# bastienjacquet/CudaDepthMapIntegration

Measured on AMD Instinct MI355X. Metric: Gvoxel-projections/s, higher is better.
Workload: dtype f64

## Files before the change

cudadepthmapintegration_amd/capi.py:

```python
from __future__ import annotations

import ctypes
import os
import sys
from typing import NamedTuple

import numpy as np

from . import build as _build
from .scene import GridDesc, RayPotential, Views

DMI_OK = 0
DMI_F32, DMI_F64 = 0, 1
DMI_DEPTH_AUTO, DMI_DEPTH_F32, DMI_DEPTH_F64 = 0, 1, 2
DMI_COMPONENTS_MIN_TRIANGLES, DMI_COMPONENTS_LARGEST = 0, 1

VARIANT_EXACT_DIVISION = 1
VARIANT_GENERAL_K = 2
VARIANT_FORCE_GENERAL = 16
VARIANT_NO_BRICK_CLASSES = 256
VARIANT_KEEP_BEHIND_ADDS = 1024
VARIANT_NO_INTERIOR = 2048
VARIANT_XCD_RUNS = 8192
VARIANT_ZMAJOR_SLOTS = 16384
VARIANT_PERSISTENT_ALWAYS = 32768
VARIANT_PERSISTENT_NEVER = 65536
VARIANT_NO_WINDOWS = 262144
VARIANT_WINDOWS_ALWAYS = 524288
VARIANT_COST_ORDER = 1048576
VARIANT_NO_COST_ORDER = 2097152
VARIANT_BRICK_CLASSES_ALWAYS = 131072
VARIANT_FIXED_TILE_SHAPE = 4096
VARIANT_SPATIAL_ORDER = 512
VARIANT_TILE_SHAPE = {"tk16_w5_g8_1x1": 0, "tk8_w6_g8_2x2": 32, "tk16_w5_g8_2x2": 64, "tk8_w6": 96, "tk8_w7_g8": 128, "tk16_w5_g4": 160,
                      "tk16_w6_g2": 192, "tk8_w6_g8_1x1": 224}


class GridDescC(ctypes.Structure):
    _fields_ = [("cell_dims", ctypes.c_int32 * 3), ("origin", ctypes.c_double * 3),
                ("spacing", ctypes.c_double * 3), ("grid_matrix", ctypes.c_double * 16)]


class RayPotentialC(ctypes.Structure):
    _fields_ = [("thickness", ctypes.c_double), ("rho", ctypes.c_double), ("eta", ctypes.c_double),
                ("delta", ctypes.c_double)]


class OptionsC(ctypes.Structure):
    _fields_ = [("device", ctypes.c_int32), ("grid_dtype", ctypes.c_int32), ("depth_storage", ctypes.c_int32),
                ("count_hits", ctypes.c_int32), ("kernel_variant", ctypes.c_int32), ("z_first", ctypes.c_int32),
                ("stream", ctypes.c_void_p), ("external_grid", ctypes.c_void_p)]


class TimingsC(ctypes.Structure):
    _fields_ = [("last_fuse_kernel_ms", ctypes.c_double), ("total_fuse_kernel_ms", ctypes.c_double),
                ("fuse_launches", ctypes.c_uint64), ("last_upload_ms", ctypes.c_double),
                ("last_download_ms", ctypes.c_double), ("last_cell_to_point_ms", ctypes.c_double),
                ("last_fuse_main_kernel_ms", ctypes.c_double), ("total_fuse_main_kernel_ms", ctypes.c_double)]


class InfoC(ctypes.Structure):
    _fields_ = [("n_voxels", ctypes.c_int64), ("n_views", ctypes.c_int32), ("depth_width", ctypes.c_int32),
                ("depth_height", ctypes.c_int32), ("depth_storage_in_use", ctypes.c_int32),
                ("grid_dtype", ctypes.c_int32), ("k_mode", ctypes.c_int32), ("kernel_variant", ctypes.c_int32),
                ("tiled_kernel", ctypes.c_int32), ("device_bytes", ctypes.c_uint64), ("pixels_without_depth", ctypes.c_uint64)]


class MultiOptionsC(ctypes.Structure):
    _fields_ = [("grid_dtype", ctypes.c_int32), ("depth_storage", ctypes.c_int32), ("kernel_variant", ctypes.c_int32),
                ("partition", ctypes.c_int32), ("exchange", ctypes.c_int32), ("n_slabs", ctypes.c_int32)]


class MultiInfoC(ctypes.Structure):
    _fields_ = [("world", ctypes.c_int32), ("n_local", ctypes.c_int32), ("first_rank", ctypes.c_int32),
                ("rccl_ranks", ctypes.c_int32), ("rccl_version", ctypes.c_int32), ("partition", ctypes.c_int32),
                ("exchange", ctypes.c_int32), ("n_slabs", ctypes.c_int32), ("n_voxels", ctypes.c_int64),
                ("n_views_total", ctypes.c_int64), ("n_views_local", ctypes.c_int64)]


class MultiTimingsC(ctypes.Structure):
    _fields_ = [("last_step_ms", ctypes.c_double), ("last_fuse_kernel_ms", ctypes.c_double),
                ("total_step_ms", ctypes.c_double), ("steps", ctypes.c_uint64)]


DMI_PARTITION_VIEWS, DMI_PARTITION_Z_SLABS = 0, 1
DMI_EXCHANGE_ALL_REDUCE, DMI_EXCHANGE_REDUCE_SCATTER, DMI_EXCHANGE_PEER_COPY = 0, 1, 2
DMI_UNIQUE_ID_BYTES = 128

ABI_SYMBOLS = [
    "dmi_default_options", "dmi_create", "dmi_destroy", "dmi_last_error", "dmi_add_views", "dmi_add_views_f32",
    "dmi_clear_views", "dmi_reset_grid", "dmi_upload_grid", "dmi_fuse", "dmi_fuse_range", "dmi_fuse_slab", "dmi_fuse_range_download", "dmi_synchronize",
    "dmi_download_grid_f64", "dmi_download_grid_f32", "dmi_download_hits", "dmi_grid_device_pointer",
    "dmi_get_brick_class_histogram", "dmi_get_timings", "dmi_get_info", "dmi_alloc_pinned", "dmi_free_pinned", "dmi_pcie_probe", "dmi_fp64_probe", "dmi_abi_version", "dmi_device_count",
    "dmi_color_mesh", "dmi_color_last_error", "dmi_cell_to_point", "dmi_download_point_data_f64",
    "dmi_point_data_device_pointer", "dmi_color_create", "dmi_color_destroy", "dmi_color_add_views",
    "dmi_color_clear_views", "dmi_color_process", "dmi_color_get_kernel_ms", "dmi_get_mixed_reason_histogram", "dmi_get_window_pair_count", "dmi_get_view_paths", "dmi_get_upload_kernel_ms", "dmi_sizeof_info", "dmi_sizeof_timings",
    "dmi_color_set_scratch_budget", "dmi_color_set_vertex_reorder", "dmi_color_add_views_with_depth", "dmi_color_set_depth_test",
    "dmi_iso_active_cells",
    "dmi_extract_isosurface", "dmi_download_isosurface", "dmi_get_isosurface_kernel_ms",
    "dmi_extract_isosurface_normals", "dmi_download_isosurface_normals",
    "dmi_filter_isosurface_components", "dmi_download_isosurface_regions", "dmi_get_isosurface_filter_kernel_ms",
    "dmi_get_isosurface_filter_pass_ms", "dmi_get_isosurface_filter_cas_retries",
    "dmi_smooth_isosurface", "dmi_get_isosurface_smooth_kernel_ms", "dmi_get_isosurface_smooth_pass_ms",
    "dmi_multi_default_options", "dmi_multi_view_shard", "dmi_multi_z_slab", "dmi_multi_slab_ranges", "dmi_multi_peer_chunk", "dmi_multi_create",
    "dmi_multi_get_unique_id", "dmi_multi_create_rank", "dmi_multi_destroy", "dmi_multi_last_error", "dmi_multi_add_views",
    "dmi_multi_add_views_f32", "dmi_multi_add_local_views", "dmi_multi_add_local_views_f32", "dmi_multi_clear_views", "dmi_multi_fuse", "dmi_multi_synchronize",
    "dmi_multi_download_grid_f32", "dmi_multi_download_grid_f64", "dmi_multi_get_info", "dmi_multi_get_timings",
    "dmi_multi_local_context",
]

_lib = None


class DmiError(RuntimeError):
    def __init__(self, code: int, message: str):
        super().__init__(f"dmi error {code}: {message}")
        self.code = code


def library_path() -> str:
    return _build.LIB_PATH


def load() -> ctypes.CDLL:
    global _lib
    if _lib is not None:
        return _lib
    if "torch" not in sys.modules:
        try:
            import torch
        except Exception:
            pass
    path = _build.build()
    if not os.path.exists(path):
        raise RuntimeError(f"{path} is missing: the HIP extension is required, there is no CPU fallback")
    L = ctypes.CDLL(path)
    vp, i32, dbl = ctypes.c_void_p, ctypes.c_int32, ctypes.c_double
    dp = ctypes.POINTER(ctypes.c_double)
    L.dmi_default_options.argtypes = [ctypes.POINTER(OptionsC)]
    L.dmi_default_options.restype = None
    L.dmi_create.argtypes = [ctypes.POINTER(GridDescC), ctypes.POINTER(RayPotentialC), ctypes.POINTER(OptionsC),
                             ctypes.POINTER(vp)]
    L.dmi_destroy.argtypes = [vp]
    L.dmi_destroy.restype = None
    L.dmi_last_error.argtypes = [vp]
    L.dmi_last_error.restype = ctypes.c_char_p
    L.dmi_add_views.argtypes = [vp, dp, dp, dbl, dp, dp, i32, i32, i32]
    L.dmi_add_views_f32.argtypes = [vp, ctypes.POINTER(ctypes.c_float), dp, dp, i32, i32, i32]
    L.dmi_clear_views.argtypes = [vp]
    L.dmi_reset_grid.argtypes = [vp]
    L.dmi_upload_grid.argtypes = [vp, dp]
    L.dmi_fuse.argtypes = [vp]
    L.dmi_fuse_range.argtypes = [vp, i32, i32]
    L.dmi_fuse_slab.argtypes = [vp, i32, i32]
    if hasattr(L, "dmi_fuse_range_download"):
        L.dmi_fuse_range_download.argtypes = [vp, i32, i32, vp, i32, i32]
    L.dmi_synchronize.argtypes = [vp]
    L.dmi_download_grid_f64.argtypes = [vp, dp]
    L.dmi_download_grid_f32.argtypes = [vp, ctypes.POINTER(ctypes.c_float)]
    L.dmi_download_hits.argtypes = [vp, ctypes.POINTER(ctypes.c_uint32), ctypes.POINTER(ctypes.c_uint64)]
    L.dmi_grid_device_pointer.argtypes = [vp, ctypes.POINTER(vp)]
    L.dmi_cell_to_point.argtypes = [vp]
    L.dmi_download_point_data_f64.argtypes = [vp, dp]
    L.dmi_point_data_device_pointer.argtypes = [vp, ctypes.POINTER(vp)]
    if hasattr(L, "dmi_iso_active_cells"):
        L.dmi_iso_active_cells.argtypes = [vp, ctypes.c_double, ctypes.POINTER(ctypes.c_uint64), ctypes.POINTER(ctypes.c_int64),
                                           ctypes.c_uint64]
    if hasattr(L, "dmi_extract_isosurface"):
        L.dmi_extract_isosurface.argtypes = [vp, ctypes.c_double, ctypes.POINTER(ctypes.c_uint64), ctypes.POINTER(ctypes.c_uint64)]
        L.dmi_download_isosurface.argtypes = [vp, dp, ctypes.POINTER(ctypes.c_int64)]
        L.dmi_get_isosurface_kernel_ms.argtypes = [vp, dp]
    if hasattr(L, "dmi_extract_isosurface_normals"):
        L.dmi_extract_isosurface_normals.argtypes = [vp, ctypes.c_double, ctypes.POINTER(ctypes.c_uint64), ctypes.POINTER(ctypes.c_uint64)]
        L.dmi_download_isosurface_normals.argtypes = [vp, ctypes.POINTER(ctypes.c_float)]
    if hasattr(L, "dmi_filter_isosurface_components"):
        u64p = ctypes.POINTER(ctypes.c_uint64)
        L.dmi_filter_isosurface_components.argtypes = [vp, ctypes.c_int, ctypes.c_uint64, u64p, u64p, u64p, u64p]
        L.dmi_download_isosurface_regions.argtypes = [vp, ctypes.POINTER(ctypes.c_int64), ctypes.POINTER(ctypes.c_int64)]
        L.dmi_get_isosurface_filter_kernel_ms.argtypes = [vp, dp]
        L.dmi_get_isosurface_filter_pass_ms.argtypes = [vp, dp]
        L.dmi_get_isosurface_filter_cas_retries.argtypes = [vp, u64p]
    if hasattr(L, "dmi_smooth_isosurface"):
        L.dmi_smooth_isosurface.argtypes = [vp, i32, dbl, dbl]
        L.dmi_get_isosurface_smooth_kernel_ms.argtypes = [vp, dp]
        L.dmi_get_isosurface_smooth_pass_ms.argtypes = [vp, dp]
    L.dmi_get_brick_class_histogram.argtypes = [vp, ctypes.POINTER(ctypes.c_uint64)]
    L.dmi_get_mixed_reason_histogram.argtypes = [vp, ctypes.POINTER(ctypes.c_uint64)]
    if hasattr(L, "dmi_get_window_pair_count"):
        L.dmi_get_window_pair_count.argtypes = [vp, ctypes.POINTER(ctypes.c_uint64)]
    if hasattr(L, "dmi_get_view_paths"):
        L.dmi_get_view_paths.argtypes = [vp, ctypes.POINTER(ctypes.c_uint64)]
    if hasattr(L, "dmi_get_upload_kernel_ms"):
        L.dmi_get_upload_kernel_ms.argtypes = [vp, dp, dp]
    for name in ("dmi_sizeof_info", "dmi_sizeof_timings"):
        if hasattr(L, name):
            getattr(L, name).restype = ctypes.c_size_t
    L.dmi_get_timings.argtypes = [vp, ctypes.POINTER(TimingsC)]
    L.dmi_get_info.argtypes = [vp, ctypes.POINTER(InfoC)]
    L.dmi_alloc_pinned.argtypes = [ctypes.c_size_t, ctypes.POINTER(vp)]
    L.dmi_free_pinned.argtypes = [vp]
    L.dmi_pcie_probe.argtypes = [i32, ctypes.c_size_t, dp, dp]
    L.dmi_fp64_probe.argtypes = [i32, ctypes.c_double, dp]
    u8p = ctypes.POINTER(ctypes.c_uint8)
    L.dmi_color_mesh.argtypes = [dp, ctypes.c_int64, u8p, dp, dp, i32, i32, i32, i32, u8p, u8p, ctypes.POINTER(ctypes.c_int32)]
    L.dmi_color_create.argtypes = [i32, ctypes.POINTER(vp)]
    L.dmi_color_destroy.argtypes = [vp]
    L.dmi_color_destroy.restype = None
    L.dmi_color_add_views.argtypes = [vp, u8p, dp, dp, i32, i32, i32]
    L.dmi_color_clear_views.argtypes = [vp]
    L.dmi_color_process.argtypes = [vp, dp, ctypes.c_int64, u8p, u8p, ctypes.POINTER(ctypes.c_int32)]
    L.dmi_color_get_kernel_ms.argtypes = [vp, dp]
    L.dmi_color_set_scratch_budget.argtypes = [vp, ctypes.c_uint64]
    L.dmi_color_set_vertex_reorder.argtypes = [vp, i32]
    L.dmi_color_add_views_with_depth.argtypes = [vp, u8p, dp, dp, dp, i32, i32, i32]
    L.dmi_color_set_depth_test.argtypes = [vp, i32, ctypes.c_double]
    L.dmi_color_last_error.argtypes = []
    L.dmi_color_last_error.restype = ctypes.c_char_p
    i64, i64p, i32p = ctypes.c_int64, ctypes.POINTER(ctypes.c_int64), ctypes.POINTER(ctypes.c_int32)
    L.dmi_multi_default_options.argtypes = [ctypes.POINTER(MultiOptionsC)]
    L.dmi_multi_default_options.restype = None
    L.dmi_multi_view_shard.argtypes = [i64, i32, i32, i64p, i64p]
    L.dmi_multi_z_slab.argtypes = [i32, i32, i32, i32p, i32p]
    L.dmi_multi_slab_ranges.argtypes = [i32, i32, i32p, i32p, i32]
    if hasattr(L, "dmi_multi_peer_chunk"):
        L.dmi_multi_peer_chunk.argtypes = [i64, i32, i32, i64p, i64p]
    L.dmi_multi_create.argtypes = [ctypes.POINTER(GridDescC), ctypes.POINTER(RayPotentialC), ctypes.POINTER(MultiOptionsC),
                                   i32p, i32, ctypes.POINTER(vp)]
    L.dmi_multi_get_unique_id.argtypes = [u8p]
    L.dmi_multi_create_rank.argtypes = [ctypes.POINTER(GridDescC), ctypes.POINTER(RayPotentialC), ctypes.POINTER(MultiOptionsC),
                                        i32, i32, i32, u8p, ctypes.POINTER(vp)]
    L.dmi_multi_destroy.argtypes = [vp]
    L.dmi_multi_destroy.restype = None
    L.dmi_multi_last_error.argtypes = [vp]
    L.dmi_multi_last_error.restype = ctypes.c_char_p
    L.dmi_multi_add_views.argtypes = [vp, dp, dp, dbl, dp, dp, i32, i32, i32]
    L.dmi_multi_add_views_f32.argtypes = [vp, ctypes.POINTER(ctypes.c_float), dp, dp, i32, i32, i32]
    L.dmi_multi_add_local_views.argtypes = [vp, i32, dp, dp, dbl, dp, dp, i32, i32, i32]
    L.dmi_multi_add_local_views_f32.argtypes = [vp, i32, ctypes.POINTER(ctypes.c_float), dp, dp, i32, i32, i32]
    L.dmi_multi_clear_views.argtypes = [vp]
    L.dmi_multi_fuse.argtypes = [vp]
    L.dmi_multi_synchronize.argtypes = [vp]
    L.dmi_multi_download_grid_f32.argtypes = [vp, ctypes.POINTER(ctypes.c_float), i64p, i64p]
    L.dmi_multi_download_grid_f64.argtypes = [vp, dp, i64p, i64p]
    L.dmi_multi_get_info.argtypes = [vp, ctypes.POINTER(MultiInfoC)]
    L.dmi_multi_get_timings.argtypes = [vp, ctypes.POINTER(MultiTimingsC)]
    L.dmi_multi_local_context.argtypes = [vp, i32, ctypes.POINTER(vp)]
    from . import build as _b
    for name in ABI_SYMBOLS:
        if _b.LIB_OVERRIDE and not hasattr(L, name):
            continue
        fn = getattr(L, name)
        if fn.restype is ctypes.c_int:
            fn.restype = ctypes.c_int
    _lib = L
    return L


def pinned_empty(shape, dtype) -> np.ndarray:
    L = load()
    n = int(np.prod(shape)) * np.dtype(dtype).itemsize
    p = ctypes.c_void_p()
    rc = L.dmi_alloc_pinned(n, ctypes.byref(p))
    if rc != DMI_OK:
        raise DmiError(rc, "dmi_alloc_pinned failed")
    buf = (ctypes.c_char * n).from_address(p.value)
    return np.frombuffer(buf, dtype=dtype).reshape(shape)


def pcie_probe(device: int = 0, n_bytes: int = 256 << 20) -> tuple[float, float]:
    L = load()
    a, b = ctypes.c_double(), ctypes.c_double()
    rc = L.dmi_pcie_probe(int(device), int(n_bytes), ctypes.byref(a), ctypes.byref(b))
    if rc != DMI_OK:
        raise DmiError(rc, L.dmi_last_error(None).decode())
    return float(a.value), float(b.value)


def fp64_probe(device: int = 0, milliseconds: float = 20.0) -> float:
    L = load()
    a = ctypes.c_double()
    rc = L.dmi_fp64_probe(int(device), float(milliseconds), ctypes.byref(a))
    if rc != DMI_OK:
        raise DmiError(rc, L.dmi_last_error(None).decode())
    return float(a.value)


def device_count() -> int:
    return int(load().dmi_device_count())


def _dp(a):
    return a.ctypes.data_as(ctypes.POINTER(ctypes.c_double))


class FusionContext:

    def __init__(self, grid: GridDesc, ray: RayPotential, *, device: int = 0, grid_dtype: str = "f64",
                 depth_storage: str = "auto", count_hits: bool = False, kernel_variant: int = 0,
                 stream: int | None = None, external_grid: int | None = None, z_first: int = 0):
        self._lib = load()
        self._h = ctypes.c_void_p()
        g = _grid_c(grid)
        r = RayPotentialC(float(ray.thickness), float(ray.rho), float(ray.eta), float(ray.delta))
        o = OptionsC()
        self._lib.dmi_default_options(ctypes.byref(o))
        o.device = device
        o.grid_dtype = {"f32": DMI_F32, "f64": DMI_F64}[grid_dtype]
        o.depth_storage = {"auto": DMI_DEPTH_AUTO, "f32": DMI_DEPTH_F32, "f64": DMI_DEPTH_F64}[depth_storage]
        o.count_hits = 1 if count_hits else 0
        o.kernel_variant = int(kernel_variant)
        o.z_first = int(z_first)
        o.stream = stream
        o.external_grid = external_grid
        self.grid = grid
        self.grid_dtype = grid_dtype
        self.n_voxels = grid.n_voxels
        self._mesh_counts = None
        rc = self._lib.dmi_create(ctypes.byref(g), ctypes.byref(r), ctypes.byref(o), ctypes.byref(self._h))
        if rc != DMI_OK:
            self._h = ctypes.c_void_p()
            raise DmiError(rc, self._lib.dmi_last_error(None).decode())

    def _check(self, rc: int):
        if rc != DMI_OK:
            raise DmiError(rc, self._lib.dmi_last_error(self._h).decode())

    def close(self):
        if getattr(self, "_h", None) is not None and self._h:
            self._lib.dmi_destroy(self._h)
            self._h = ctypes.c_void_p()

    def __enter__(self):
        return self

    def __exit__(self, *exc):
        self.close()

    def __del__(self):
        try:
            self.close()
        except Exception:
            pass
# ... 57 lines not shown

    def download_grid(self, dtype=np.float64, out: np.ndarray | None = None) -> np.ndarray:
        nx, ny, nz = (int(c) for c in self.grid.cell_dims)
        if out is None:
            out = np.empty(self.n_voxels, dtype=dtype)
        if out.dtype != np.dtype(dtype) or out.size != self.n_voxels or not out.flags.c_contiguous:
            raise ValueError("out must be a contiguous array of n_voxels elements of the requested dtype")
        if np.dtype(dtype) == np.float64:
            self._check(self._lib.dmi_download_grid_f64(self._h, _dp(out)))
        else:
            self._check(self._lib.dmi_download_grid_f32(self._h, out.ctypes.data_as(ctypes.POINTER(ctypes.c_float))))
        return out.reshape(nz, ny, nx)

    def download_hits(self):
        nx, ny, nz = (int(c) for c in self.grid.cell_dims)
        vh = np.empty(self.n_voxels, dtype=np.uint32)
        mh = np.empty(self.info().n_views, dtype=np.uint64)
        self._check(self._lib.dmi_download_hits(self._h, vh.ctypes.data_as(ctypes.POINTER(ctypes.c_uint32)),
                                                mh.ctypes.data_as(ctypes.POINTER(ctypes.c_uint64))))
        return vh.reshape(nz, ny, nx), mh

    def grid_device_pointer(self) -> int:
        p = ctypes.c_void_p()
        self._check(self._lib.dmi_grid_device_pointer(self._h, ctypes.byref(p)))
        return int(p.value)

    def cell_to_point(self):
        self._check(self._lib.dmi_cell_to_point(self._h))

    def download_point_data(self) -> np.ndarray:
        nx, ny, nz = (int(c) for c in self.grid.cell_dims)
        out = np.empty((nz + 1) * (ny + 1) * (nx + 1), dtype=np.float64)
        self._check(self._lib.dmi_download_point_data_f64(self._h, _dp(out)))
        return out.reshape(nz + 1, ny + 1, nx + 1)

    def iso_active_cells(self, iso: float, ids: bool = True):
        n = ctypes.c_uint64(0)
        self._check(self._lib.dmi_iso_active_cells(self._h, float(iso), ctypes.byref(n), None, 0))
        if not ids:
            return int(n.value), None
        out = np.empty(int(n.value), dtype=np.int64)
        if n.value:
            self._check(self._lib.dmi_iso_active_cells(self._h, float(iso), ctypes.byref(n),
                                                       out.ctypes.data_as(ctypes.POINTER(ctypes.c_int64)), out.size))
        return int(n.value), out

    def extract_isosurface(self, iso: float):
        nv, nt = ctypes.c_uint64(0), ctypes.c_uint64(0)
        self._mesh_counts = None
        self._check(self._lib.dmi_extract_isosurface(self._h, float(iso), ctypes.byref(nv), ctypes.byref(nt)))
        verts = np.empty((max(int(nv.value), 1), 3), dtype=np.float64)
        tris = np.empty((max(int(nt.value), 1), 3), dtype=np.int64)
        self._mesh_counts = (int(nv.value), int(nt.value), 0)
        self._check(self._lib.dmi_download_isosurface(self._h, _dp(verts), tris.ctypes.data_as(ctypes.POINTER(ctypes.c_int64))))
        return verts[:int(nv.value)], tris[:int(nt.value)]

    def extract_isosurface_with_normals(self, iso: float):
        nv, nt = ctypes.c_uint64(0), ctypes.c_uint64(0)
        self._mesh_counts = None
        self._check(self._lib.dmi_extract_isosurface_normals(self._h, float(iso), ctypes.byref(nv), ctypes.byref(nt)))
        verts = np.empty((max(int(nv.value), 1), 3), dtype=np.float64)
        tris = np.empty((max(int(nt.value), 1), 3), dtype=np.int64)
        normals = np.empty((max(int(nv.value), 1), 3), dtype=np.float32)
        self._mesh_counts = (int(nv.value), int(nt.value), 0)
        self._check(self._lib.dmi_download_isosurface(self._h, _dp(verts), tris.ctypes.data_as(ctypes.POINTER(ctypes.c_int64))))
        self._check(self._lib.dmi_download_isosurface_normals(self._h, normals.ctypes.data_as(ctypes.POINTER(ctypes.c_float))))
        return verts[:int(nv.value)], tris[:int(nt.value)], normals[:int(nv.value)]

    def filter_isosurface_components(self, mode: str = "min_triangles", min_triangles: int = 0):
        m = {"min_triangles": DMI_COMPONENTS_MIN_TRIANGLES, "largest": DMI_COMPONENTS_LARGEST}[mode]
        out = [ctypes.c_uint64(0) for _ in range(4)]
        self._check(self._lib.dmi_filter_isosurface_components(self._h, m, int(min_triangles), *[ctypes.byref(x) for x in out]))
        self._mesh_counts = (int(out[0].value), int(out[1].value), int(out[3].value))
        return tuple(int(x.value) for x in out)

    def _current_mesh_counts(self):
        c = self._mesh_counts
        if c is None:
            raise DmiError(1, "no mesh: extract_isosurface has not succeeded")
        return c

    def download_isosurface(self):
        nv, nt, _ = self._current_mesh_counts()
        verts = np.empty((max(nv, 1), 3), dtype=np.float64)
        tris = np.empty((max(nt, 1), 3), dtype=np.int64)
        self._check(self._lib.dmi_download_isosurface(self._h, _dp(verts), tris.ctypes.data_as(ctypes.POINTER(ctypes.c_int64))))
        return verts[:nv], tris[:nt]

    def download_isosurface_normals(self):
        nv, _, _ = self._current_mesh_counts()
        normals = np.empty((max(nv, 1), 3), dtype=np.float32)
        self._check(self._lib.dmi_download_isosurface_normals(self._h, normals.ctypes.data_as(ctypes.POINTER(ctypes.c_float))))
        return normals[:nv]

    def download_isosurface_regions(self):
        nv, _, nk = self._current_mesh_counts()
        rid = np.empty(max(nv, 1), dtype=np.int64)
        rsz = np.empty(max(nk, 1), dtype=np.int64)
        i64p = ctypes.POINTER(ctypes.c_int64)
        self._check(self._lib.dmi_download_isosurface_regions(self._h, rid.ctypes.data_as(i64p), rsz.ctypes.data_as(i64p)))
        return rid[:nv], rsz[:nk]

    def isosurface_filter_kernel_ms(self) -> float:
        a = ctypes.c_double(0)
        self._check(self._lib.dmi_get_isosurface_filter_kernel_ms(self._h, ctypes.byref(a)))
        return float(a.value)

    def isosurface_filter_cas_retries(self) -> int:
        a = ctypes.c_uint64(0)
        self._check(self._lib.dmi_get_isosurface_filter_cas_retries(self._h, ctypes.byref(a)))
        return int(a.value)

    def isosurface_filter_pass_ms(self) -> dict:
        a = (ctypes.c_double * 4)()
        self._check(self._lib.dmi_get_isosurface_filter_pass_ms(self._h, a))
        return dict(zip(("labels", "sizes", "scans", "compaction"), (float(x) for x in a)))

    def smooth_isosurface(self, iterations: int, lam: float = 0.5, mu: float = -0.53) -> None:
        self._check(self._lib.dmi_smooth_isosurface(self._h, int(iterations), float(lam), float(mu)))

    def isosurface_smooth_kernel_ms(self) -> float:
        a = ctypes.c_double(0)
        self._check(self._lib.dmi_get_isosurface_smooth_kernel_ms(self._h, ctypes.byref(a)))
        return float(a.value)

    def isosurface_smooth_pass_ms(self) -> dict:
        a = (ctypes.c_double * 3)()
        self._check(self._lib.dmi_get_isosurface_smooth_pass_ms(self._h, a))
        return dict(zip(("adjacency", "steps", "normals"), (float(x) for x in a)))

    def isosurface_kernel_ms(self) -> float:
        a = ctypes.c_double(0)
        self._check(self._lib.dmi_get_isosurface_kernel_ms(self._h, ctypes.byref(a)))
        return float(a.value)

    def brick_class_histogram(self) -> dict:
        h = (ctypes.c_uint64 * 4)()
        self._check(self._lib.dmi_get_brick_class_histogram(self._h, h))
        return {"mixed": int(h[0]), "free": int(h[1]), "behind": int(h[2]), "skip": int(h[3])}

    def mixed_reason_histogram(self) -> dict:
        h = (ctypes.c_uint64 * 8)()
        self._check(self._lib.dmi_get_mixed_reason_histogram(self._h, h))
        names = ["unspecified", "degenerate", "camera_plane", "image_border", "nan_depth", "sentinel_and_depth", "near_surface",
                 "free_or_no_depth"]
        return {n: int(h[i]) for i, n in enumerate(names)}

    def window_pair_count(self) -> int:
        n = ctypes.c_uint64(0)
        if not hasattr(self._lib, "dmi_get_window_pair_count"):
            return 0
        self._check(self._lib.dmi_get_window_pair_count(self._h, ctypes.byref(n)))
        return int(n.value)

    def upload_kernel_ms(self) -> tuple:
        if not hasattr(self._lib, "dmi_get_upload_kernel_ms"):
            return (0.0, 0.0)
        a, b = ctypes.c_double(0), ctypes.c_double(0)
        self._check(self._lib.dmi_get_upload_kernel_ms(self._h, ctypes.byref(a), ctypes.byref(b)))
        return (float(a.value), float(b.value))

    def timings(self) -> TimingsC:
        t = TimingsC()
        self._check(self._lib.dmi_get_timings(self._h, ctypes.byref(t)))
        return t

    def info(self) -> InfoC:
        i = InfoC()
        self._check(self._lib.dmi_get_info(self._h, ctypes.byref(i)))
        return i

    def view_paths(self) -> dict:
        names = ("general_kernel", "tiled_general_k", "tiled_fp64_selection", "tiled_tier1", "tiled_tier1_per_lane_margin", "with_window_record")
        if not hasattr(self._lib, "dmi_get_view_paths"):
            return {}
        a = (ctypes.c_uint64 * 6)()
        self._check(self._lib.dmi_get_view_paths(self._h, a))
        return {k: int(v) for k, v in zip(names, a)}


def _grid_c(grid: GridDesc) -> GridDescC:
    g = GridDescC()
    for i in range(3):
        g.cell_dims[i] = int(grid.cell_dims[i])
        g.origin[i] = float(grid.origin[i])
        g.spacing[i] = float(grid.spacing[i])
    gm = np.ascontiguousarray(grid.grid_matrix, dtype=np.float64).reshape(16)
    for i in range(16):
        g.grid_matrix[i] = gm[i]
    return g


def multi_view_shard(n: int, rank: int, world: int) -> tuple[int, int]:
    a, b = ctypes.c_int64(), ctypes.c_int64()
    if load().dmi_multi_view_shard(int(n), int(rank), int(world), ctypes.byref(a), ctypes.byref(b)) != DMI_OK:
        raise ValueError("rank/world out of range")
    return int(a.value), int(a.value + b.value)


def multi_z_slab(nz: int, rank: int, world: int) -> tuple[int, int]:
    a, b = ctypes.c_int32(), ctypes.c_int32()
    if load().dmi_multi_z_slab(int(nz), int(rank), int(world), ctypes.byref(a), ctypes.byref(b)) != DMI_OK:
        raise ValueError("rank/world out of range")
    return int(a.value), int(a.value + b.value)


def multi_peer_chunk(n: int, world: int, c: int) -> tuple[int, int]:
    a, b = ctypes.c_int64(), ctypes.c_int64()
    rc = load().dmi_multi_peer_chunk(int(n), int(world), int(c), ctypes.byref(a), ctypes.byref(b))
    if rc != DMI_OK:
        raise DmiError(rc, "dmi_multi_peer_chunk: invalid argument")
    return int(a.value), int(b.value)


def multi_slab_ranges(nz: int, n_slabs: int) -> list[tuple[int, int]]:
    a, b = (ctypes.c_int32 * 64)(), (ctypes.c_int32 * 64)()
    n = load().dmi_multi_slab_ranges(int(nz), int(n_slabs), a, b, 64)
    return [(int(a[i]), int(b[i])) for i in range(n)]


def multi_unique_id() -> bytes:
    L = load()
    buf = (ctypes.c_uint8 * DMI_UNIQUE_ID_BYTES)()
    rc = L.dmi_multi_get_unique_id(buf)
    if rc != DMI_OK:
        raise DmiError(rc, L.dmi_multi_last_error(None).decode())
    return bytes(buf)


class MultiContext:

    def __init__(self, grid: GridDesc, ray: RayPotential, *, devices=None, rank: int | None = None, world: int | None = None,
                 unique_id: bytes | None = None, device: int = 0, grid_dtype: str = "f32", depth_storage: str = "auto",
                 kernel_variant: int = 0, partition: str = "views", exchange: str = "all_reduce", n_slabs: int = 0):
        self._lib = load()
        self._h = ctypes.c_void_p()
        o = MultiOptionsC()
        self._lib.dmi_multi_default_options(ctypes.byref(o))
        o.grid_dtype = {"f32": DMI_F32, "f64": DMI_F64}[grid_dtype]
        o.depth_storage = {"auto": DMI_DEPTH_AUTO, "f32": DMI_DEPTH_F32, "f64": DMI_DEPTH_F64}[depth_storage]
        o.kernel_variant = int(kernel_variant)
        o.partition = {"views": DMI_PARTITION_VIEWS, "z_slabs": DMI_PARTITION_Z_SLABS}[partition]
        o.exchange = {"all_reduce": DMI_EXCHANGE_ALL_REDUCE, "reduce_scatter": DMI_EXCHANGE_REDUCE_SCATTER,
                      "peer_copy": DMI_EXCHANGE_PEER_COPY}[exchange]
        o.n_slabs = int(n_slabs)
        g = _grid_c(grid)
        r = RayPotentialC(float(ray.thickness), float(ray.rho), float(ray.eta), float(ray.delta))
        self.grid = grid
        self.grid_dtype = grid_dtype
        self.n_voxels = grid.n_voxels
        if devices is not None:
            d = (ctypes.c_int32 * len(devices))(*[int(x) for x in devices])
            rc = self._lib.dmi_multi_create(ctypes.byref(g), ctypes.byref(r), ctypes.byref(o), d, len(devices), ctypes.byref(self._h))
        else:
            if rank is None or world is None:
                raise ValueError("MultiContext needs devices=[...] or rank= and world=")
            idbuf = None
            if unique_id is not None:
                if len(unique_id) != DMI_UNIQUE_ID_BYTES:
                    raise ValueError("unique_id must be 128 bytes")
                idbuf = (ctypes.c_uint8 * DMI_UNIQUE_ID_BYTES).from_buffer_copy(unique_id)
            rc = self._lib.dmi_multi_create_rank(ctypes.byref(g), ctypes.byref(r), ctypes.byref(o), int(device), int(rank),
                                                 int(world), idbuf, ctypes.byref(self._h))
        if rc != DMI_OK:
            self._h = ctypes.c_void_p()
            raise DmiError(rc, self._lib.dmi_multi_last_error(None).decode())

    def _check(self, rc: int):
        if rc != DMI_OK:
            raise DmiError(rc, self._lib.dmi_multi_last_error(self._h).decode())

    def close(self):
        if getattr(self, "_h", None) is not None and self._h:
            self._lib.dmi_multi_destroy(self._h)
            self._h = ctypes.c_void_p()

    def __enter__(self):
        return self

    def __exit__(self, *exc):
        self.close()

    def __del__(self):
        try:
            self.close()
        except Exception:
            pass

    def add_views(self, views: Views, threshold: float | None = None, local_index: int | None = None):
        n, H, W = views.depth.shape
        K4 = np.ascontiguousarray(views.K4, dtype=np.float64).reshape(n, 16)
        RT4 = np.ascontiguousarray(views.RT4, dtype=np.float64).reshape(n, 16)
        L = self._lib
        if views.depth.dtype == np.float32:
            d = np.ascontiguousarray(views.depth)
            dptr = d.ctypes.data_as(ctypes.POINTER(ctypes.c_float))
            if local_index is None:
                self._check(L.dmi_multi_add_views_f32(self._h, dptr, _dp(K4), _dp(RT4), n, W, H))
            else:
                self._check(L.dmi_multi_add_local_views_f32(self._h, int(local_index), dptr, _dp(K4), _dp(RT4), n, W, H))
            return
        d = np.ascontiguousarray(views.depth, dtype=np.float64)
        bc = None
        if views.best_cost is not None and threshold is not None:
            bc = np.ascontiguousarray(views.best_cost, dtype=np.float64)
        thr = float(threshold) if threshold is not None else 0.0
# ... 585 lines not shown
```

cudadepthmapintegration_amd/csrc/dmi_capi.hip:

```cpp
#include "../../include/dmi.h"
#include "fusion_kernels.h"

#include <chrono>
#include <cmath>
#include <cstdio>
#include <cstdlib>
#include <cstring>
#include <exception>
#include <limits>
#include <new>
#include <string>
#include <vector>

using dmi::FuseArgs;
using dmi::FuseConfig;
using dmi::MapRec;
using dmi::TileArgs;
using dmi::TileMapRec;

namespace {

thread_local std::string g_create_error;

struct Batch {
// ... 1111 lines not shown
  std::vector<std::pair<uint64_t, int32_t>> keyed(n);
  size_t q = 0;
  for (int32_t z = 0; z < super_z; ++z)
    for (int32_t y = 0; y < super_y; ++y)
      for (int32_t x = 0; x < super_x; ++x, ++q)
        keyed[q] = {zmajor ? (uint64_t)q : (spread(x) | (spread(y) << 1) | (spread(z) << 2)), x | (y << 10) | (z << 20)};
  if (!zmajor) std::sort(keyed.begin(), keyed.end());
  std::vector<int32_t> perm(n);
  for (size_t i = 0; i < n; ++i) perm[i] = keyed[i].second;
  int32_t *d = nullptr;
  DMI_HIP(ctx, hipMalloc(&d, n * sizeof(int32_t)));
  hipError_t e = hipMemcpyAsync(d, perm.data(), n * sizeof(int32_t), hipMemcpyHostToDevice, ctx->stream);
  if (e != hipSuccess) {
    (void)hipFree(d);
    return fail(ctx, DMI_ERR_DEVICE, std::string("slot permutation upload: ") + hipGetErrorString(e));
  }
  if (ctx->slot_perms.size() >= 64) {
    DMI_HIP(ctx, hipStreamSynchronize(ctx->stream));
    for (auto &sp : ctx->slot_perms) {
      (void)hipFree(sp.d_perm);
      ctx->device_bytes -= (uint64_t)sp.super_x * sp.super_y * sp.super_z * sizeof(int32_t);
    }
    ctx->slot_perms.clear();
  }
  ctx->slot_perms.push_back({super_x, super_y, super_z, zmajor ? 1 : 0, d});
  ctx->device_bytes += n * sizeof(int32_t);
  *out = d;
  return DMI_OK;
}

int fuse_run(dmi_context *ctx, int32_t first, int32_t count, int32_t z_first, int32_t z_count, bool tiled, int run_k_mode,
             bool general_k) {
  const int32_t n_views = (int32_t)ctx->h_maps.size();
  DMI_HIP(ctx, hipSetDevice(ctx->opt.device));
  int rc = sync_maps(ctx);
  if (rc != DMI_OK) return rc;
  const bool whole_grid = z_first == 0 && z_count == ctx->grid.cell_dims[2];
  if (!whole_grid) {
    rc = flush_zero_fill(ctx);
    if (rc != DMI_OK) return rc;
  }

  FuseArgs a;
  std::memset(&a, 0, sizeof(a));
  a.nx = ctx->grid.cell_dims[0];
  a.ny = ctx->grid.cell_dims[1];
  a.nz = ctx->grid.cell_dims[2];
  a.W = ctx->W;
  a.H = ctx->H;
  a.first_map = first;
  a.n_maps = count;
  a.init_from_grid = 0;
  for (int32_t z = z_first; z < z_first + z_count; ++z)
    if (!ctx->layer_is_zero[(size_t)z]) a.init_from_grid = 1;
  a.kz0 = ctx->opt.z_first;
  a.k_first = z_first;
  a.k_count = z_count;
  a.ox = ctx->grid.origin[0];
  a.oy = ctx->grid.origin[1];
  a.oz = ctx->grid.origin[2];
  a.sx = ctx->grid.spacing[0];
  a.sy = ctx->grid.spacing[1];
  a.sz = ctx->grid.spacing[2];
  std::memcpy(a.g, ctx->grid.grid_matrix, 12 * sizeof(double));
  a.thick = ctx->ray.thickness;
  a.delta = ctx->ray.delta;
  a.rho_pos = ctx->ray.rho * 1.0;
  a.rho_neg = ctx->ray.rho * -1.0;
  a.rho_zero = ctx->ray.rho * 0.0;
  a.slope = ctx->ray.rho / ctx->ray.thickness;
  a.free_space = -ctx->ray.eta * ctx->ray.rho;
  a.maps = ctx->d_maps;
  a.grid = ctx->d_grid;
  a.voxel_hits = ctx->d_voxel_hits;
  a.map_hits = ctx->d_map_hits;

  FuseConfig cfg;
  cfg.depth_is_f64 = ctx->depth_f64 ? 1 : 0;
  cfg.grid_is_f64 = ctx->opt.grid_dtype == DMI_F64 ? 1 : 0;
  cfg.k_mode = run_k_mode;
  cfg.count_hits = ctx->opt.count_hits ? 1 : 0;
  cfg.variant = ctx->opt.kernel_variant;

  cfg.use_tile = tiled ? 1 : 0;
  cfg.general_k = tiled && general_k ? 1 : 0;
  bool tall_by_holes = false, many_borders = false;
  {
    unsigned long long mingled = 0, strips = 0, without = 0;
    for (const Batch &bt : ctx->batches) {
      mingled += bt.mingled_strips;
      without += bt.holes;
      strips += (unsigned long long)bt.n * (unsigned long long)ctx->W * (unsigned long long)(ctx->H / 8);
    }
    const bool scattered = without <= 6 * mingled;
    cfg.holes = scattered && mingled * 160 > strips ? 1 : 0;
    tall_by_holes = scattered && mingled * 80 > strips;
    many_borders = mingled * 25 > strips;
    tall_by_holes = tall_by_holes || many_borders;
  }
  bool mostly_empty = false;
  if (!cfg.holes) {
    unsigned long long without = 0, pixels = 0;
    for (const Batch &bt : ctx->batches) {
      without += bt.holes;
      pixels += (unsigned long long)bt.n * (unsigned long long)ctx->W * (unsigned long long)ctx->H;
    }
    mostly_empty = without * 4 >= pixels && pixels > 0;
  }
  if (cfg.use_tile && !(cfg.variant & (dmi::VAR_TILE_SHAPE_MASK | dmi::VAR_FIXED_TILE_SHAPE))) {
    const int64_t bricks16 = (int64_t)((a.nx + 15) / 16) * ((a.ny + 15) / 16) * ((a.nz + 15) / 16);
    if (bricks16 <= 32768 && !(tall_by_holes && bricks16 >= 4096) && !(mostly_empty && bricks16 >= 13824))
      cfg.variant |= 7 << dmi::VAR_TILE_SHAPE_SHIFT;
  }

  TileArgs t;
  std::memset(&t, 0, sizeof(t));
  if (cfg.use_tile) {
    const dmi::TileShape sh = dmi::tile_shape(cfg.variant, ctx->depth_f64, !grid_axis_aligned(ctx->grid), cfg.general_k != 0);
    t.nx = a.nx; t.ny = a.ny; t.nz = a.nz; t.W = a.W; t.H = a.H;
    t.first_map = first; t.n_maps = count; t.init_from_grid = a.init_from_grid;
    t.kpad = (a.nz + sh.tk - 1) / sh.tk * sh.tk;
    t.bricks_x = (a.nx + 8 * sh.wx - 1) / (8 * sh.wx);
    t.bricks_y = (a.ny + 8 * sh.wy - 1) / (8 * sh.wy);
    t.bricks_z = t.kpad / sh.tk;
    t.super_x = (t.bricks_x + 3) / 4;
    t.super_y = (t.bricks_y + 3) / 4;
    t.super_z = (t.bricks_z + 1) / 2;
    if (!whole_grid) {
      t.sbz_first = z_first / (2 * sh.tk);
      t.super_z = (z_first + z_count + 2 * sh.tk - 1) / (2 * sh.tk) - t.sbz_first;
    }
    if (t.bricks_x > 2047 || t.bricks_y > 2047 || t.bricks_z > 1023)
      return fail(ctx, DMI_ERR_INVALID_ARGUMENT, "dmi_fuse: more bricks along an axis than the tiled kernel's order entries hold");
    t.slot_base = t.sbz_first * t.super_x * t.super_y * 32;
    t.slot_count = t.super_x * t.super_y * t.super_z * 32;
    rc = slot_permutation(ctx, t.super_x, t.super_y, t.super_z, (cfg.variant & dmi::VAR_ZMAJOR_SLOTS) != 0, &t.sb_perm);
    if (rc != DMI_OK) return rc;
    t.xcd_run_wg = 32 * std::max(1, t.super_x * t.super_y);
    if (((int64_t)t.super_x * t.super_y * t.super_z * 32 + 16 * (int64_t)t.xcd_run_wg + 64) > (int64_t)0x7fffffff)
      return fail(ctx, DMI_ERR_INVALID_ARGUMENT, "dmi_fuse: grid too large for one launch");
    t.depth_bytes = (int32_t)((int64_t)a.W * a.H * (ctx->depth_f64 ? 8 : 4));
    t.kz0 = a.kz0;
#ifdef DMI_TUNING
    if (std::getenv("DMI_DEBUG_NO_DEPTH_LOADS")) t.depth_bytes = 0;
#endif
    t.ox = a.ox; t.oy = a.oy; t.oz = a.oz; t.sx = a.sx; t.sy = a.sy; t.sz = a.sz;
    std::memcpy(t.g, a.g, sizeof(t.g));
    t.thick = a.thick; t.delta = a.delta; t.rho_pos = a.rho_pos; t.rho_neg = a.rho_neg;
    t.slope = a.slope; t.free_space = a.free_space;
    t.tile_maps = ctx->d_tile_maps;
    t.grid = a.grid; t.voxel_hits = a.voxel_hits; t.map_hits = a.map_hits;
    t.rotated = grid_axis_aligned(ctx->grid) ? 0 : 1;
    t.flags = ((cfg.variant & dmi::VAR_NO_INTERIOR) ? dmi::TILE_FLAG_NO_INTERIOR : 0) |
              ((cfg.variant & dmi::VAR_XCD_RUNS) ? dmi::TILE_FLAG_XCD_RUNS : 0);
    t.maps = ctx->d_maps;
    const size_t table_doubles = std::max<size_t>((size_t)n_views, 4) * (size_t)t.kpad;
    const size_t need = table_doubles + (size_t)dmi::kFreeSumsMax + 1;
    if (ctx->cz_table_capacity < need) {
      if (ctx->d_cz_table) {
        DMI_HIP(ctx, hipStreamSynchronize(ctx->stream));
        (void)hipFree(ctx->d_cz_table);
        ctx->device_bytes -= ctx->cz_table_capacity * 8;
        ctx->d_cz_table = nullptr;
        ctx->cz_table_capacity = 0;
      }
      const size_t grown = need * 2;
      DMI_HIP(ctx, hipMalloc(&ctx->d_cz_table, grown * 8));
      ctx->cz_table_capacity = grown;
      ctx->device_bytes += grown * 8;
    }
    t.cz_table = ctx->d_cz_table;
    if (!ctx->d_queue_heads) DMI_HIP(ctx, hipMalloc(&ctx->d_queue_heads, 128 * sizeof(int32_t)));
    t.queue_heads = ctx->d_queue_heads;
    if (!a.init_from_grid && !ctx->opt.count_hits && count <= dmi::kFreeSumsMax) t.free_sums = ctx->d_cz_table + table_doubles;
    t.wbricks_x = (a.nx + 7) / 8;
    t.wbricks_y = (a.ny + 7) / 8;
    if (!(cfg.variant & (dmi::VAR_NO_BRICK_CLASSES | dmi::VAR_BRICK_CLASSES_ALWAYS)) &&
        (int64_t)t.wbricks_x * t.wbricks_y * (int64_t)t.bricks_z <= dmi::kNoClassesMaxBricks && count < dmi::kNoClassesMaxViews)
      cfg.variant |= dmi::VAR_NO_BRICK_CLASSES;
    t.class_pitch = 64;
    while (t.class_pitch < n_views) t.class_pitch *= 2;
    if (cfg.variant & dmi::VAR_NO_BRICK_CLASSES) {
      if (ctx->zero_row_capacity < (size_t)t.class_pitch) {
        if (ctx->d_zero_row) {
          DMI_HIP(ctx, hipStreamSynchronize(ctx->stream));
          (void)hipFree(ctx->d_zero_row);
          ctx->d_zero_row = nullptr;
        }
        DMI_HIP(ctx, hipMalloc(&ctx->d_zero_row, (size_t)t.class_pitch));
        DMI_HIP(ctx, hipMemsetAsync(ctx->d_zero_row, dmi::BRICK_MIXED, (size_t)t.class_pitch, ctx->stream));
        ctx->zero_row_capacity = (size_t)t.class_pitch;
      }
      t.classes = ctx->d_zero_row;
      t.class_pitch = 0;
    } else {
      const size_t fine_bytes = ((size_t)t.wbricks_x * t.wbricks_y * t.bricks_z * (size_t)t.class_pitch + 255) / 256 * 256;
      const size_t coarse_end = (fine_bytes + (size_t)dmi::coarse_class_bytes(t, sh.tk) + 255) / 256 * 256;
      bool any_tier1 = false;
      for (int32_t m = first; m < first + count && !any_tier1; ++m) any_tier1 = std::isfinite(ctx->h_win_recs[(size_t)m].e_abs);
      const bool zero_free = (!a.init_from_grid || ctx->grid_free_of_negative_zero) && !ctx->opt.count_hits && !(cfg.variant & dmi::VAR_KEEP_BEHIND_ADDS);
      const bool windows = DMI_TIER1 != 0 && !cfg.general_k && !cfg.count_hits && !(cfg.variant & (dmi::VAR_NO_WINDOWS | dmi::VAR_NO_INTERIOR)) &&
                           (cfg.holes || many_borders || (cfg.variant & dmi::VAR_WINDOWS_ALWAYS)) && any_tier1 && zero_free && !ctx->depth_f64;
      const size_t cbytes = coarse_end + (windows ? fine_bytes * sizeof(dmi::WinPair) : 0);
      ctx->coarse_offset = fine_bytes;
      if (ctx->classes_capacity < cbytes) {
        if (ctx->d_classes) {
          DMI_HIP(ctx, hipStreamSynchronize(ctx->stream));
          (void)hipFree(ctx->d_classes);
          ctx->device_bytes -= ctx->classes_capacity;
          ctx->d_classes = nullptr;
          ctx->classes_capacity = 0;
        }
        DMI_HIP(ctx, hipMalloc(&ctx->d_classes, cbytes));
        DMI_HIP(ctx, hipMemsetAsync(ctx->d_classes, dmi::BRICK_SKIP, cbytes, ctx->stream));
        ctx->classes_capacity = cbytes;
        ctx->device_bytes += cbytes;
      }
      t.classes = ctx->d_classes;
      if (windows) {
        t.win_origin = reinterpret_cast<dmi::WinPair *>(ctx->d_classes + coarse_end);
        t.win_delta = (int64_t)reinterpret_cast<intptr_t>(t.win_origin) - 16 * (int64_t)reinterpret_cast<intptr_t>(t.classes);
        t.win_recs = ctx->d_win_recs;
        t.foot_recs = ctx->d_foot_recs;
        t.vb_bytes = (int32_t)std::min<int64_t>(dmi::valid_bits_bytes(ctx->W, ctx->H), 0x7fffffff);
        t.vb_rowskip = (dmi::valid_bits_tiles_x(ctx->W) - 1) * 128;
        t.win_cx = dmi::kValidMargin + ctx->W / 2;
        t.win_cy = dmi::kValidMargin + ctx->H / 2;
      }
      if (!(cfg.variant & dmi::VAR_SPATIAL_ORDER)) {
        const size_t n_slots = (size_t)t.super_x * t.super_y * t.super_z * 32;
        if (ctx->order_capacity < n_slots) {
          if (ctx->d_order) {
            DMI_HIP(ctx, hipStreamSynchronize(ctx->stream));
            (void)hipFree(ctx->d_order);
            (void)hipFree(ctx->d_order_level);
            ctx->device_bytes -= ctx->order_capacity * 5 + 4;
            ctx->d_order = nullptr;
            ctx->d_order_level = nullptr;
            ctx->order_capacity = 0;
          }
          DMI_HIP(ctx, hipMalloc(&ctx->d_order, (n_slots + 1) * sizeof(int32_t)));
          DMI_HIP(ctx, hipMalloc(&ctx->d_order_level, dmi::order_scratch_bytes(n_slots)));
          ctx->order_capacity = n_slots;
          ctx->device_bytes += n_slots * 5 + 4;
        }
        t.order = ctx->d_order + 1;
        t.n_order = ctx->d_order;
        t.order_levels = reinterpret_cast<const int32_t *>(ctx->d_order_level + (n_slots + 15) / 16 * 16);
        t.xcd_run_wg = 32 * (4 / (sh.wx * sh.wy));
        const bool cost_order = sh.wx * sh.wy == 1 && !(cfg.variant & dmi::VAR_NO_COST_ORDER) &&
                                ((cfg.variant & dmi::VAR_COST_ORDER) || n_slots <= (size_t)dmi::kCostOrderMaxSlots);
        if (cost_order) {
          t.flags |= dmi::TILE_FLAG_COST_ORDER | dmi::TILE_FLAG_XCD_RUNS;
          t.xcd_run_wg = 16;
        }
      }
    }
    if ((!a.init_from_grid || ctx->grid_free_of_negative_zero) && !ctx->opt.count_hits && !(cfg.variant & dmi::VAR_KEEP_BEHIND_ADDS))
      t.behind_mask = 0x0101010101010101ull;
#ifdef DMI_TUNING
    if (std::getenv("DMI_DEBUG_WG_TIMES")) {
      const size_t per_round = 8 * (size_t)t.xcd_run_wg;
      const size_t blocks = ((size_t)t.super_x * t.super_y * t.super_z * 32 + 32 + per_round - 1) / per_round * per_round;
      if (ctx->wg_times_blocks < blocks) {
        if (ctx->d_wg_times) {
          DMI_HIP(ctx, hipStreamSynchronize(ctx->stream));
          (void)hipFree(ctx->d_wg_times);
        }
        DMI_HIP(ctx, hipMalloc(&ctx->d_wg_times, blocks * 3 * sizeof(unsigned long long)));
        ctx->wg_times_blocks = blocks;
      }
      DMI_HIP(ctx, hipMemsetAsync(ctx->d_wg_times, 0, blocks * 3 * sizeof(unsigned long long), ctx->stream));
      t.wg_times = ctx->d_wg_times;
      t.wg_times_n = (int64_t)blocks;
    }
    if (const char *e = std::getenv("DMI_DEBUG_PAIRS")) {
      if (!std::strcmp(e, "nowin")) t.flags |= dmi::TILE_FLAG_DBG_SKIP_WINDOW_PAIRS;
      if (!std::strcmp(e, "onlywin")) t.flags |= dmi::TILE_FLAG_DBG_ONLY_WINDOW_PAIRS;
      if (!std::strcmp(e, "nowinloads")) t.flags |= dmi::TILE_FLAG_DBG_NO_WINDOW_LOADS;
    }
    if (const char *e = std::getenv("DMI_XCD_RUN_WG")) {
      t.xcd_run_wg = std::max(1, std::atoi(e));
      if (((int64_t)t.super_x * t.super_y * t.super_z * 32 + 8 * (int64_t)t.xcd_run_wg) > (int64_t)0x7fffffff)
        return fail(ctx, DMI_ERR_INVALID_ARGUMENT, "dmi_fuse: DMI_XCD_RUN_WG makes the launch too large");
    }
#endif
    if (!ctx->d_fuse_args) DMI_HIP(ctx, hipMalloc(&ctx->d_fuse_args, sizeof(FuseArgs)));
    DMI_HIP(ctx, hipMemcpyAsync(ctx->d_fuse_args, &a, sizeof(FuseArgs), hipMemcpyHostToDevice, ctx->stream));
    t.full = ctx->d_fuse_args;
  }

  EventPair ev;
  if (!ctx->pool.empty()) {
    ev = ctx->pool.back();
    ctx->pool.pop_back();
  } else {
    DMI_HIP(ctx, hipEventCreate(&ev.start));
    DMI_HIP(ctx, hipEventCreate(&ev.stop));
    DMI_HIP(ctx, hipEventCreate(&ev.mid));
  }
  ev.has_mid = cfg.use_tile != 0 && !(cfg.variant & dmi::VAR_NO_BRICK_CLASSES);
  DMI_HIP(ctx, hipEventRecord(ev.start, ctx->stream));
  hipError_t e = cfg.use_tile ? dmi::launch_fuse_tiled(t, ctx->d_maps, cfg, ctx->pyramid, ctx->d_order_level,
                                                         ctx->d_classes ? ctx->d_classes + ctx->coarse_offset : nullptr,
                                                         ev.has_mid ? ev.mid : nullptr, ctx->stream) : dmi::launch_fuse(a, cfg, ctx->stream);
  if (e != hipSuccess) {
    ctx->pool.push_back(ev);
// ... 670 lines not shown
      rc = ensure_buffer(ctx, (void **)&ctx->d_mesh_alt_normals, &cap, nv * 12);
      if (rc != DMI_OK) return rc;
      ctx->mesh_alt_normal_capacity = cap / 12;
    }
    rc = ensure_buffer(ctx, (void **)&ctx->d_smooth_keys, &ctx->smooth_keys_capacity, 2 * std::max<uint64_t>(6 * nt, 2) * 8);
    if (rc != DMI_OK) return rc;
    rc = ensure_buffer(ctx, &ctx->d_smooth_vertex_scratch, &ctx->smooth_vertex_scratch_capacity, fixed_words * 8 + 3 * (nv + 1) * 4);
    if (rc != DMI_OK) return rc;
  }
  size_t temp_bytes = 0;
  DMI_HIP(ctx, dmi::smooth_temp_bytes(nv, nt, &temp_bytes));
  temp_bytes = std::max<size_t>(temp_bytes, 16);
  rc = ensure_buffer(ctx, &ctx->d_smooth_temp, &ctx->smooth_temp_capacity, temp_bytes);
  if (rc != DMI_OK) return rc;
  if (!ctx->smooth_events[0])
    for (hipEvent_t &e : ctx->smooth_events) DMI_HIP(ctx, hipEventCreate(&e));
  dmi::SmoothMesh m{};
  m.n_vertices = nv;
  m.n_triangles = nt;
  m.vertices = ctx->d_mesh_vertices;
  m.triangles = ctx->d_mesh_triangles;
  m.normals_out = normals ? ctx->d_mesh_alt_normals : nullptr;
  dmi::SmoothScratch s{};
  s.keys[0] = ctx->d_smooth_keys;
  s.keys[1] = ctx->d_smooth_keys + std::max<uint64_t>(6 * nt, 2);
  s.fixed = (unsigned long long *)ctx->d_smooth_vertex_scratch;
  s.row_start = (uint32_t *)(s.fixed + fixed_words);
  s.valence = s.row_start + (nv + 1);
  s.offsets = s.valence + (nv + 1);
  s.positions[0] = ctx->d_mesh_alt_vertices;
  s.positions[1] = ctx->d_smooth_vertices;
  s.temp = ctx->d_smooth_temp;
  s.temp_bytes = temp_bytes;
  double *result = nullptr;
  DMI_HIP(ctx, dmi::launch_isosurface_smooth(m, s, iterations, lambda, mu, &result, ctx->smooth_events, ctx->stream));
  DMI_HIP(ctx, hipStreamSynchronize(ctx->stream));
  float ms = 0.f;
  DMI_HIP(ctx, hipEventElapsedTime(&ms, ctx->smooth_events[0], ctx->smooth_events[3]));
  ctx->last_smooth_kernel_ms = (double)ms;
  for (int p = 0; p < 3; ++p) {
    DMI_HIP(ctx, hipEventElapsedTime(&ms, ctx->smooth_events[p], ctx->smooth_events[p + 1]));
    ctx->last_smooth_pass_ms[p] = (double)ms;
  }
  if (result == ctx->d_mesh_alt_vertices) {
    std::swap(ctx->d_mesh_vertices, ctx->d_mesh_alt_vertices);
    std::swap(ctx->mesh_vertex_capacity, ctx->mesh_alt_vertex_capacity);
  } else {
    std::swap(ctx->d_mesh_vertices, ctx->d_smooth_vertices);
    std::swap(ctx->mesh_vertex_capacity, ctx->smooth_vertex_capacity);
  }
  if (normals) {
    std::swap(ctx->d_mesh_normals, ctx->d_mesh_alt_normals);
    std::swap(ctx->mesh_normal_capacity, ctx->mesh_alt_normal_capacity);
  }
  return DMI_OK;
  });
}

int dmi_get_isosurface_smooth_kernel_ms(dmi_context *ctx, double *last) {
  return guarded(ctx, "dmi_get_isosurface_smooth_kernel_ms", [&]() -> int {
  if (!ctx || !last) return fail(ctx, DMI_ERR_INVALID_ARGUMENT, "dmi_get_isosurface_smooth_kernel_ms: null argument");
  *last = ctx->last_smooth_kernel_ms;
  return DMI_OK;
  });
}

int dmi_get_isosurface_smooth_pass_ms(dmi_context *ctx, double out[3]) {
  return guarded(ctx, "dmi_get_isosurface_smooth_pass_ms", [&]() -> int {
  if (!ctx || !out) return fail(ctx, DMI_ERR_INVALID_ARGUMENT, "dmi_get_isosurface_smooth_pass_ms: null argument");
  for (int p = 0; p < 3; ++p) out[p] = ctx->last_smooth_pass_ms[p];
  return DMI_OK;
  });
}

int dmi_get_brick_class_histogram(dmi_context *ctx, uint64_t out[4]) {
  return guarded(ctx, "dmi_get_brick_class_histogram", [&]() -> int {
  if (!ctx || !out) return fail(ctx, DMI_ERR_INVALID_ARGUMENT, "dmi_get_brick_class_histogram: null argument");
  out[0] = out[1] = out[2] = out[3] = 0;
  if (!ctx->last_fuse_classes) return DMI_OK;
  DMI_HIP(ctx, hipSetDevice(ctx->opt.device));
  const size_t bytes = (size_t)ctx->last_class_bricks * ctx->last_class_pitch;
  std::vector<uint8_t> host(bytes);
  DMI_HIP(ctx, hipMemcpyAsync(host.data(), ctx->d_classes, bytes, hipMemcpyDeviceToHost, ctx->stream));
  DMI_HIP(ctx, hipStreamSynchronize(ctx->stream));
  for (int64_t b = 0; b < ctx->last_class_bricks; ++b) {
    const uint8_t *row = host.data() + (size_t)b * ctx->last_class_pitch + ctx->last_first;
    for (int32_t m = 0; m < ctx->last_count; ++m) out[row[m] & 3] += 1;
  }
  return DMI_OK;
  });
}

int dmi_get_mixed_reason_histogram(dmi_context *ctx, uint64_t out[8]) {
  return guarded(ctx, "dmi_get_mixed_reason_histogram", [&]() -> int {
  if (!ctx || !out) return fail(ctx, DMI_ERR_INVALID_ARGUMENT, "dmi_get_mixed_reason_histogram: null argument");
  for (int i = 0; i < 8; ++i) out[i] = 0;
  if (!ctx->last_fuse_classes) return DMI_OK;
  DMI_HIP(ctx, hipSetDevice(ctx->opt.device));
  const size_t bytes = (size_t)ctx->last_class_bricks * ctx->last_class_pitch;
  std::vector<uint8_t> host(bytes);
  DMI_HIP(ctx, hipMemcpyAsync(host.data(), ctx->d_classes, bytes, hipMemcpyDeviceToHost, ctx->stream));
  DMI_HIP(ctx, hipStreamSynchronize(ctx->stream));
  for (int64_t b = 0; b < ctx->last_class_bricks; ++b) {
    const uint8_t *row = host.data() + (size_t)b * ctx->last_class_pitch + ctx->last_first;
    for (int32_t m = 0; m < ctx->last_count; ++m)
      if ((row[m] & 3) == dmi::BRICK_MIXED) out[(row[m] >> 2) & 7] += 1;
  }
  return DMI_OK;
  });
}

int dmi_get_view_paths(dmi_context *ctx, uint64_t out[6]) {
  return guarded(ctx, "dmi_get_view_paths", [&]() -> int {
  if (!ctx || !out) return fail(ctx, DMI_ERR_INVALID_ARGUMENT, "dmi_get_view_paths: null argument");
  for (int i = 0; i < 6; ++i) out[i] = 0;
  const bool possible = tile_eligible(ctx);
  for (size_t m = 0; m < ctx->h_maps.size(); ++m) {
    const TileMapRec &t = ctx->h_tile_maps[m];
    if (!possible || !ctx->view_tile_ok[m]) {
      out[0] += 1;
    } else if (ctx->view_k_mode[m] == dmi::K_GENERAL) {
      out[1] += 1;
    } else {
      out[2 + std::min(std::max(t.t1_ok, 0), 2)] += 1;
      if (t.t1_ok != 0 && std::isfinite(ctx->h_win_recs[m].e_abs)) out[5] += 1;
    }
  }
  return DMI_OK;
  });
}

int dmi_get_window_pair_count(dmi_context *ctx, uint64_t *out) {
  return guarded(ctx, "dmi_get_window_pair_count", [&]() -> int {
  if (!ctx || !out) return fail(ctx, DMI_ERR_INVALID_ARGUMENT, "dmi_get_window_pair_count: null argument");
  *out = 0;
  if (!ctx->last_fuse_classes || !ctx->last_win_origin) return DMI_OK;
  DMI_HIP(ctx, hipSetDevice(ctx->opt.device));
  const size_t pairs = (size_t)ctx->last_class_bricks * ctx->last_class_pitch;
  std::vector<uint8_t> host(pairs);
  DMI_HIP(ctx, hipMemcpyAsync(host.data(), ctx->d_classes, pairs, hipMemcpyDeviceToHost, ctx->stream));
  DMI_HIP(ctx, hipStreamSynchronize(ctx->stream));
  const int64_t per_layer = ctx->last_class_bricks / std::max<int64_t>(1, ctx->last_bricks_z);
  for (int64_t b = 0; b < ctx->last_class_bricks; ++b) {
    const int64_t bz = b / std::max<int64_t>(1, per_layer);
    if (bz * ctx->last_tk + ctx->last_tk > ctx->grid.cell_dims[2]) continue;
    const size_t base = (size_t)b * ctx->last_class_pitch + ctx->last_first;
    for (int32_t m = 0; m < ctx->last_count; ++m)
      if ((host[base + m] & 0x3f) == (dmi::BRICK_MIXED | (dmi::MIXED_FREE_OR_NODEPTH << 2))) *out += 1;
  }
  return DMI_OK;
  });
}

int dmi_get_timings(dmi_context *ctx, dmi_timings *out) {
  return guarded(ctx, "dmi_get_timings", [&]() -> int {
  if (!ctx || !out) return fail(ctx, DMI_ERR_INVALID_ARGUMENT, "dmi_get_timings: null argument");
  DMI_HIP(ctx, hipSetDevice(ctx->opt.device));
  int rc = drain_events(ctx);
  if (rc != DMI_OK) return rc;
  rc = drain_c2p(ctx);
  if (rc != DMI_OK) return rc;
  *out = ctx->timings;
  return DMI_OK;
  });
}

int dmi_get_info(dmi_context *ctx, dmi_info *out) {
  return guarded(ctx, "dmi_get_info", [&]() -> int {
  if (!ctx || !out) return fail(ctx, DMI_ERR_INVALID_ARGUMENT, "dmi_get_info: null argument");
  std::memset(out, 0, sizeof(*out));
  out->n_voxels = ctx->n_voxels;
  out->n_views = (int32_t)ctx->h_maps.size();
  out->depth_width = ctx->W;
  out->depth_height = ctx->H;
  out->depth_storage_in_use = ctx->depth_f64 ? DMI_DEPTH_F64 : DMI_DEPTH_F32;
  out->grid_dtype = ctx->opt.grid_dtype;
  out->k_mode = (ctx->opt.kernel_variant & 2) ? 0 : ctx->k_mode;
  out->kernel_variant = ctx->opt.kernel_variant;
  bool all_tiled = !ctx->h_maps.empty() && tile_eligible(ctx);
  for (uint8_t ok : ctx->view_tile_ok) all_tiled = all_tiled && ok;
  out->tiled_kernel = all_tiled ? 1 : 0;
  out->device_bytes = ctx->device_bytes;
  for (const Batch &bt : ctx->batches) out->pixels_without_depth += bt.holes;
  return DMI_OK;
  });
}

int dmi_alloc_pinned(size_t bytes, void **out) {
  return guarded(nullptr, "dmi_alloc_pinned", [&]() -> int {
  if (!out || bytes == 0) return DMI_ERR_INVALID_ARGUMENT;
  hipError_t e = hipHostMalloc(out, bytes, hipHostMallocDefault);
  if (e != hipSuccess) {
    (void)hipGetLastError();
    g_create_error = std::string("dmi_alloc_pinned: ") + hipGetErrorString(e);
    return e == hipErrorOutOfMemory ? DMI_ERR_OUT_OF_MEMORY : DMI_ERR_DEVICE;
  }
  return DMI_OK;
  });
}

int dmi_pcie_probe(int32_t device, size_t bytes, double *h2d_GBps, double *d2h_GBps) {
  return guarded(nullptr, "dmi_pcie_probe", [&]() -> int {
    if (bytes < (size_t(1) << 20) || (!h2d_GBps && !d2h_GBps))
      return fail(nullptr, DMI_ERR_INVALID_ARGUMENT, "dmi_pcie_probe: at least 1 MiB and one output");
    dmi_context *none = nullptr;
    DMI_HIP(none, hipSetDevice(device));
    void *host = nullptr, *dev = nullptr;
    hipStream_t s = nullptr;
    hipEvent_t e0 = nullptr, e1 = nullptr;
    hipError_t e = hipHostMalloc(&host, bytes, hipHostMallocDefault);
    if (e == hipSuccess) e = hipMalloc(&dev, bytes);
    if (e == hipSuccess) e = hipStreamCreateWithFlags(&s, hipStreamNonBlocking);
    if (e == hipSuccess) e = hipEventCreate(&e0);
    if (e == hipSuccess) e = hipEventCreate(&e1);
    double rate[2] = {0.0, 0.0};
    if (e == hipSuccess) std::memset(host, 0, bytes);
    for (int dir = 0; e == hipSuccess && dir < 2; ++dir) {
      for (int rep = 0; e == hipSuccess && rep < 3; ++rep) {
        e = hipEventRecord(e0, s);
        if (e == hipSuccess)
          e = dir == 0 ? hipMemcpyAsync(dev, host, bytes, hipMemcpyHostToDevice, s) : hipMemcpyAsync(host, dev, bytes, hipMemcpyDeviceToHost, s);
        if (e == hipSuccess) e = hipEventRecord(e1, s);
        if (e == hipSuccess) e = hipEventSynchronize(e1);
        float ms = 0.f;
        if (e == hipSuccess) e = hipEventElapsedTime(&ms, e0, e1);
        if (e == hipSuccess && rep > 0 && ms > 0.f) rate[dir] = std::max(rate[dir], (double)bytes / (ms * 1e-3) / 1e9);
      }
    }
    if (e1) (void)hipEventDestroy(e1);
    if (e0) (void)hipEventDestroy(e0);
    if (s) (void)hipStreamDestroy(s);
    if (dev) (void)hipFree(dev);
    if (host) (void)hipHostFree(host);
    if (e != hipSuccess) {
      (void)hipGetLastError();
      return fail(nullptr, DMI_ERR_DEVICE, std::string("dmi_pcie_probe: ") + hipGetErrorString(e));
    }
    if (h2d_GBps) *h2d_GBps = rate[0];
    if (d2h_GBps) *d2h_GBps = rate[1];
    return DMI_OK;
  });
}

#ifdef DMI_TUNING
extern "C" int dmi_debug_wg_times(dmi_context *ctx, unsigned long long *out, int64_t capacity, int64_t *blocks) {
  if (!ctx || !blocks) return DMI_ERR_INVALID_ARGUMENT;
  *blocks = (int64_t)ctx->wg_times_blocks;
  if (!ctx->d_wg_times || !out || capacity < 3 * (int64_t)ctx->wg_times_blocks) return DMI_OK;
  if (hipStreamSynchronize(ctx->stream) != hipSuccess) return DMI_ERR_DEVICE;
  if (hipMemcpy(out, ctx->d_wg_times, ctx->wg_times_blocks * 3 * sizeof(unsigned long long), hipMemcpyDeviceToHost) != hipSuccess)
    return DMI_ERR_DEVICE;
  return DMI_OK;
}
#endif

int dmi_fp64_probe(int32_t device, double milliseconds, double *tflops) {
  return guarded(nullptr, "dmi_fp64_probe", [&]() -> int {
    if (!tflops || !(milliseconds > 0.0) || milliseconds > 1000.0)
      return fail(nullptr, DMI_ERR_INVALID_ARGUMENT, "dmi_fp64_probe: an output and 0 < milliseconds <= 1000");
    dmi_context *none = nullptr;
    DMI_HIP(none, hipSetDevice(device));
    hipDeviceProp_t prop;
    DMI_HIP(none, hipGetDeviceProperties(&prop, device));
    const int blocks = std::max(1, prop.multiProcessorCount) * 8;
    double *out = nullptr;
    hipStream_t s = nullptr;
    hipEvent_t e0 = nullptr, e1 = nullptr;
    hipError_t e = hipMalloc(&out, (size_t)blocks * 256 * sizeof(double));
    if (e == hipSuccess) e = hipStreamCreateWithFlags(&s, hipStreamNonBlocking);
    if (e == hipSuccess) e = hipEventCreate(&e0);
    if (e == hipSuccess) e = hipEventCreate(&e1);
    double best = 0.0;
    int iters = 4096;
    for (int rep = 0; e == hipSuccess && rep < 4; ++rep) {
      e = hipEventRecord(e0, s);
      if (e == hipSuccess) e = dmi::launch_fp64_probe(out, blocks, iters, s);
      if (e == hipSuccess) e = hipEventRecord(e1, s);
      if (e == hipSuccess) e = hipEventSynchronize(e1);
      float ms = 0.f;
      if (e == hipSuccess) e = hipEventElapsedTime(&ms, e0, e1);
      if (e != hipSuccess || !(ms > 0.f)) break;
      const double flops = 2.0 * 8.0 * (double)iters * (double)blocks * 256.0;
      if (rep > 0) best = std::max(best, flops / (ms * 1e-3) / 1e12);
      if (rep == 0) iters = (int)std::min(4.0e6, std::max(1024.0, iters * milliseconds / ms));
    }
    if (e1) (void)hipEventDestroy(e1);
    if (e0) (void)hipEventDestroy(e0);
    if (s) (void)hipStreamDestroy(s);
    if (out) (void)hipFree(out);
    if (e != hipSuccess) {
      (void)hipGetLastError();
      return fail(nullptr, DMI_ERR_DEVICE, std::string("dmi_fp64_probe: ") + hipGetErrorString(e));
    }
    *tflops = best;
    return DMI_OK;
  });
}

int dmi_free_pinned(void *ptr) {
  return guarded(nullptr, "dmi_free_pinned", [&]() -> int {
  if (!ptr) return DMI_OK;
  hipError_t e = hipHostFree(ptr);
  if (e != hipSuccess) {
    (void)hipGetLastError();
    return DMI_ERR_DEVICE;
  }
// ... 6 lines not shown
```

cudadepthmapintegration_amd/csrc/fusion_classify.hip:

```cpp
#include <algorithm>
#include <cstring>

#include <stdlib.h>

#include "fusion_kernels.h"
#include "fusion_device.h"

namespace dmi {

namespace {

template <typename T>
__device__ __forceinline__ T cload(const T *p) {
  return *reinterpret_cast<const T __attribute__((address_space(4))) *>(reinterpret_cast<uintptr_t>(p));
}

__device__ __forceinline__ float float_below(double d) {
  float f = (float)d;
  if ((double)f > d) f = nextafterf(f, -__builtin_inff());
  return f;
}
__device__ __forceinline__ float float_above(double d) {
  float f = (float)d;
  if ((double)f < d) f = nextafterf(f, __builtin_inff());
// ... 226 lines not shown
        bad = bad || !(hz == hz);
        hzmin = fmin(hzmin, hz);
        hzmax = fmax(hzmax, hz);
      }
      czmin = fmin(czmin, cz);
      czmax = fmax(czmax, cz);
      umin = fmin(umin, u);
      umax = fmax(umax, u);
      vmin = fmin(vmin, v);
      vmax = fmax(vmax, v);
    }
    czmin -= 2.0 * tr->cz_err;
    czmax += 2.0 * tr->cz_err;
  } else {
  double wxs[2], wys[2], wzs[2];
  for (int c = 0; c < 2; ++c) {
    const int i = c ? i1 : i0, j = c ? j1 : j0, k = c ? k1 : k0;
    const double gx = a.ox + (i + 0.5) * a.sx;
    const double gy = a.oy + (j + 0.5) * a.sy;
    const double gz = a.oz + ((k + a.kz0) + 0.5) * a.sz;
    wxs[c] = row4(a.g + 0, gx, gy, gz);
    wys[c] = row4(a.g + 4, gx, gy, gz);
    wzs[c] = row4(a.g + 8, gx, gy, gz);
  }
  const double r20 = mr->rt[8], r21 = mr->rt[9], r22 = mr->rt[10];
  const double zx[2] = {r20 * wxs[0], r20 * wxs[1]}, zy[2] = {r21 * wys[0], r21 * wys[1]}, zz[2] = {r22 * wzs[0], r22 * wzs[1]};
  const double ux[2] = {tr->px * wxs[0], tr->px * wxs[1]};
  const double uy[2] = {__builtin_fma(tr->py, wys[0], tr->p0), __builtin_fma(tr->py, wys[1], tr->p0)};
  const double uz[2] = {tr->pz * wzs[0], tr->pz * wzs[1]};
  const double vx[2] = {tr->qx * wxs[0], tr->qx * wxs[1]};
  const double vy[2] = {__builtin_fma(tr->qy, wys[0], tr->q0), __builtin_fma(tr->qy, wys[1], tr->q0)};
  const double vz[2] = {tr->qz * wzs[0], tr->qz * wzs[1]};
  double sxw[2] = {0.0, 0.0}, syw[2] = {0.0, 0.0}, szw[2] = {0.0, 0.0};
  if (genk) {
    sxw[0] = tr->sx * wxs[0], sxw[1] = tr->sx * wxs[1];
    syw[0] = __builtin_fma(tr->sy, wys[0], tr->s0), syw[1] = __builtin_fma(tr->sy, wys[1], tr->s0);
    szw[0] = tr->sz * wzs[0], szw[1] = tr->sz * wzs[1];
  }
#pragma unroll
  for (int c = 0; c < 8; ++c) {
    const int cx = c & 1, cy = (c >> 1) & 1, ck = c >> 2;
    const double cz = ((zx[cx] + zy[cy]) + zz[ck]) + r23;
    const double hx = (ux[cx] + uy[cy]) + uz[ck];
    const double hy = (vx[cx] + vy[cy]) + vz[ck];
    const double hz = genk ? (sxw[cx] + syw[cy]) + szw[ck] : cz;
    double r = __builtin_amdgcn_rcp(hz);
    r = __builtin_fma(r, __builtin_fma(-hz, r, 1.0), r);
    const double u = hx * r, v = hy * r;
    bad = bad || !(cz == cz);
    if (genk) {
      bad = bad || !(hz == hz);
      hzmin = fmin(hzmin, hz);
      hzmax = fmax(hzmax, hz);
    }
    czmin = fmin(czmin, cz);
    czmax = fmax(czmax, cz);
    umin = fmin(umin, u);
    umax = fmax(umax, u);
    vmin = fmin(vmin, v);
    vmax = fmax(vmax, v);
  }
  }
  uint8_t cls = BRICK_MIXED | (MIXED_DEGENERATE << 2);
  const double errz2 = 2.0 * tr->errz;
  const double err = genk ? tr->err + 65536.0 * tr->errz : tr->err;
  const double dmin = genk ? hzmin - errz2 : czmin, dmax = genk ? hzmax + errz2 : czmax;
  const double ulimit = genk ? 65536.0 : 0x1p30;
  if (!bad) {
    cls = BRICK_MIXED | (MIXED_CAMERA_PLANE << 2);
    if (dmax < 0.0) {
      cls = BRICK_SKIP;
    } else if (dmin > 4.0 * err && dmin > 0.0 && umin == umin && umax == umax && vmin == vmin && vmax == vmax &&
               fabs(umin) < ulimit && fabs(umax) < ulimit && fabs(vmin) < ulimit && fabs(vmax) < ulimit) {
      double rmin = __builtin_amdgcn_rcp(dmin);
      rmin = __builtin_fma(rmin, __builtin_fma(-dmin, rmin, 1.0), rmin);
      const double e = 2.0 * err * rmin * (1.0 + 0x1p-30) + 0x1p-20;
      const int x0 = (int)ceil(umin - 0.5 - e), x1 = (int)floor(umax + 0.5 + e);
      const int y0 = (int)ceil(vmin - 0.5 - e), y1 = (int)floor(vmax + 0.5 + e);
      cls = BRICK_MIXED | (MIXED_IMAGE_BORDER << 2);
      fp.rx0 = x0;
      fp.rx1 = x1;
      fp.ry0 = y0;
      fp.ry1 = y1;
      if (x1 < 0 || y1 < 0 || x0 >= a.W || y0 >= a.H) {
        cls = BRICK_SKIP;
      } else if (x0 >= 0 && y0 >= 0 && x1 < a.W && y1 < a.H) {
        fp.query = true;
        fp.x0 = x0;
        fp.x1 = x1;
        fp.y0 = y0;
        fp.y1 = y1;
      } else {
        fp.partial = true;
        fp.in_margin = x0 >= -kValidMargin && y0 >= -kValidMargin && x1 < a.W + kValidMargin && y1 < a.H + kValidMargin;
        fp.x0 = max(x0, 0);
        fp.x1 = min(x1, a.W - 1);
        fp.y0 = max(y0, 0);
        fp.y1 = min(y1, a.H - 1);
      }
    }
  }
  fp.cls = cls;
  fp.czmin = czmin;
  fp.czmax = czmax;
  return fp;
}

template <bool ROT, bool GK>
__device__ __forceinline__ BoxFootprint box_footprint(const TileArgs &a, const MapRec *__restrict__ mr,
                                                      const TileMapRec *__restrict__ tr, int i0, int i1, int j0, int j1, int k0,
                                                      int k1) {
  if constexpr (GK) {
    if (tr->errz != 0.0) return box_footprint_k<ROT, true>(a, mr, tr, i0, i1, j0, j1, k0, k1);
  }
  return box_footprint_k<ROT, false>(a, mr, tr, i0, i1, j0, j1, k0, k1);
}

__device__ __forceinline__ uint8_t class_from_bounds(const TileArgs &a, const TileAcc &d, double czmin, double czmax) {
  if (d.flags & TILE_HAS_NAN) return BRICK_MIXED | (MIXED_NAN_DEPTH << 2);
  if (!(d.flags & TILE_HAS_VALID)) return BRICK_SKIP;
  const bool holes = (d.flags & TILE_HAS_SENTINEL) != 0;
  if ((czmax - (double)d.dmin) < -a.delta) {
    if (!holes) return BRICK_FREE;
    const bool free_column_exact = a.behind_mask != 0 || __builtin_signbit(a.free_space);
    return free_column_exact ? (uint8_t)(BRICK_MIXED | (MIXED_FREE_OR_NODEPTH << 2)) : (uint8_t)(BRICK_MIXED | (MIXED_SENTINEL_AND_DEPTH << 2));
  }
  if ((czmin - (double)d.dmax) > a.delta) {
    if (!holes) return BRICK_BEHIND;
    return a.behind_mask ? (uint8_t)BRICK_SKIP : (uint8_t)(BRICK_MIXED | (MIXED_SENTINEL_AND_DEPTH << 2));
  }
  return BRICK_MIXED | ((holes ? MIXED_SENTINEL_AND_DEPTH : MIXED_NEAR_SURFACE) << 2);
}

template <bool GK>
__device__ __forceinline__ uint8_t border_class(const TileArgs &a, const BoxFootprint &fp, const TileAcc &d) {
  const uint8_t c = class_from_bounds(a, d, fp.czmin, fp.czmax);
  if (c == BRICK_SKIP || (c == BRICK_BEHIND && a.behind_mask)) return BRICK_SKIP;
  const bool map_serves = DMI_TIER1 != 0 && !GK && fp.in_margin && a.behind_mask != 0;
  if (map_serves && (c == BRICK_FREE || c == (uint8_t)(BRICK_MIXED | (MIXED_FREE_OR_NODEPTH << 2))))
    return BRICK_MIXED | (MIXED_FREE_OR_NODEPTH << 2);
  return BRICK_MIXED | (MIXED_IMAGE_BORDER << 2);
}

template <int kQueryTiles, bool ROT, bool GK>
__device__ __forceinline__ uint8_t classify_box(const TileArgs &a, const MapRec *__restrict__ mr,
                                                const TileMapRec *__restrict__ tr, const PyramidDesc &P, int i0, int i1,
                                                int j0, int j1, int k0, int k1) {
  const BoxFootprint fp = box_footprint<ROT, GK>(a, mr, tr, i0, i1, j0, j1, k0, k1);
  if (fp.partial) return border_class<GK>(a, fp, pyramid_query<kQueryTiles>(mr->pyramid, P, fp.x0, fp.x1, fp.y0, fp.y1));
  if (!fp.query) return fp.cls;
  return class_from_bounds(a, pyramid_query<kQueryTiles>(mr->pyramid, P, fp.x0, fp.x1, fp.y0, fp.y1), fp.czmin, fp.czmax);
}

constexpr int kCostLevels = 64;

template <bool ROT, bool GK>
__global__ __launch_bounds__(256) void classify_coarse_kernel(const TileArgs a, const MapRec *__restrict__ maps,
                                                              const PyramidDesc P, int tk, uint8_t *__restrict__ classes,
                                                              uint8_t *__restrict__ coarse) {
  fill_launch_tables(a, maps, ((int64_t)blockIdx.y * gridDim.x + blockIdx.x) * 256 + threadIdx.y * 64 + threadIdx.x,
                     (int64_t)gridDim.x * gridDim.y * 256);
  if ((a.flags & TILE_FLAG_COST_ORDER) && blockIdx.x == 0 && blockIdx.y == 0 && threadIdx.y == 0)
    for (int q = threadIdx.x; q < 2 * kCostLevels; q += 64) const_cast<int32_t *>(a.order_levels)[q] = 0;
  const int bz_first = 2 * a.sbz_first;
  const int bz_count = min(2 * a.super_z, a.bricks_z - bz_first);
  const int per_z = 32 / tk;
  const int cx_n = (a.wbricks_x + 3) / 4, cy_n = (a.wbricks_y + 3) / 4, cz_n = (bz_count + per_z - 1) / per_z;
  const int local = blockIdx.x * 4 + threadIdx.y;
  const int mm = blockIdx.y * 64 + threadIdx.x;
  if (local >= cx_n * cy_n * cz_n || mm >= a.n_maps) return;
  const int m = a.first_map + mm;
  const int cbx = local % cx_n;
  const int ct = local / cx_n;
  const int cby = ct % cy_n, cbz = ct / cy_n + bz_first / per_z;
  const int bz0 = cbz * per_z;
  const BoxFootprint fp = box_footprint<ROT, GK>(a, maps + m, a.tile_maps + m, cbx * 32, cbx * 32 + 31, cby * 32, cby * 32 + 31,
                                                 bz0 * tk, bz0 * tk + 31);
  uint8_t cls = fp.cls;
  bool speckled = false;
  if (fp.query) {
    const TileAcc d = pyramid_query<5>(maps[m].pyramid, P, fp.x0, fp.x1, fp.y0, fp.y1);
    cls = class_from_bounds(a, d, fp.czmin, fp.czmax);
    speckled = !(d.flags & (TILE_PART_HOLE_FREE | TILE_PART_NO_VALID));
  } else if (fp.partial) {
    cls = border_class<GK>(a, fp, pyramid_query<5>(maps[m].pyramid, P, fp.x0, fp.x1, fp.y0, fp.y1));
  }
  const bool inherit_mixed = cls == (uint8_t)(BRICK_MIXED | (MIXED_FREE_OR_NODEPTH << 2)) && speckled;
  coarse[(int64_t)((cbz * cy_n + cby) * cx_n + cbx) * a.class_pitch + m] = inherit_mixed ? (uint8_t)(cls | COARSE_CHILDREN_WRITTEN) : cls;
  if ((cls & 3) == BRICK_MIXED && !inherit_mixed) return;
  for (int dz = 0; dz < per_z; ++dz) {
    const int bz = bz0 + dz;
    if (bz >= bz_first + bz_count) break;
    for (int dy = 0; dy < 4; ++dy) {
      const int by = cby * 4 + dy;
      if (by >= a.wbricks_y) break;
      for (int dx = 0; dx < 4; ++dx) {
        const int bx = cbx * 4 + dx;
        if (bx >= a.wbricks_x) break;
        classes[(int64_t)((bz * a.wbricks_y + by) * a.wbricks_x + bx) * a.class_pitch + m] = cls;
      }
    }
  }
}

constexpr int kWindow = 16;

template <int kQueryTiles, int kChildren, bool ROT, bool GK>
__global__ __launch_bounds__(256) void classify_kernel(const TileArgs a, const MapRec *__restrict__ maps,
                                                       const PyramidDesc P, int tk, uint8_t *__restrict__ classes,
                                                       const uint8_t *__restrict__ coarse, int group_views) {
  constexpr int children = kChildren;
  constexpr int views_per_wave = 64 / children;
  constexpr int per_z = children / 16;
  __shared__ float2 window_mm[4 * views_per_wave][kWindow * kWindow];
  __shared__ uint8_t window_fl[4 * views_per_wave][kWindow * kWindow];
  const int bz_first = 2 * a.sbz_first;
  const int bz_count = min(2 * a.super_z, a.bricks_z - bz_first);
  const int cx_n = (a.wbricks_x + 3) / 4, cy_n = (a.wbricks_y + 3) / 4;
  const int lane = threadIdx.x & 63, wave = __builtin_amdgcn_readfirstlane(threadIdx.x >> 6);
  const int local = blockIdx.x;
  const int cbx = local % cx_n;
  const int ct = local / cx_n;
  const int cby = ct % cy_n, cbz = ct / cy_n + bz_first / per_z;
  const int chunk0 = blockIdx.y * group_views;
  const uint8_t *__restrict__ crow = coarse + (int64_t)((cbz * cy_n + cby) * cx_n + cbx) * a.class_pitch + a.first_map + chunk0;
  const unsigned long long unproven = __builtin_amdgcn_ballot_w64(
      lane < group_views && chunk0 + lane < a.n_maps && (crow[lane] & (3 | COARSE_CHILDREN_WRITTEN)) == BRICK_MIXED);
  if (unproven == 0) return;
  unsigned long long items = views_per_wave == 1 ? unproven & (0x1111111111111111ull << wave)
                                                 : (unproven | (unproven >> 1)) & (0x0101010101010101ull << (2 * wave));
  const int child = lane % children;
  const int bx = cbx * 4 + (child & 3), by = cby * 4 + ((child >> 2) & 3), bz = cbz * per_z + (child >> 4);
  const bool in_grid = bx < a.wbricks_x && by < a.wbricks_y && bz < bz_first + bz_count;
  uint8_t *__restrict__ out = classes + (int64_t)((bz * a.wbricks_y + by) * a.wbricks_x + bx) * a.class_pitch;
  while (items) {
    const int first = __builtin_ctzll(items);
    items &= items - 1;
    const int rel = first + lane / children;
    const int mm = chunk0 + rel;
    const int m = a.first_map + min(mm, a.n_maps - 1);
    const bool mine = in_grid && ((unproven >> rel) & 1ull);
    const MapRec *__restrict__ mr = maps + m;
    BoxFootprint fp;
    fp.query = false;
    fp.partial = false;
    fp.in_margin = false;
    fp.cls = BRICK_SKIP;
    MapRec mr_u;
    TileMapRec tr_u;
    if constexpr (views_per_wave == 1) {
      const int mu = __builtin_amdgcn_readfirstlane(m);
      const MapRec *src = maps + mu;
      const TileMapRec *tsrc = a.tile_maps + mu;
#pragma unroll
      for (int q = 8; q < 12; ++q) mr_u.rt[q] = cload(&src->rt[q]);
      mr_u.pyramid = cload(&src->pyramid);
      tr_u.px = cload(&tsrc->px); tr_u.py = cload(&tsrc->py); tr_u.pz = cload(&tsrc->pz); tr_u.p0 = cload(&tsrc->p0);
      tr_u.qx = cload(&tsrc->qx); tr_u.qy = cload(&tsrc->qy); tr_u.qz = cload(&tsrc->qz); tr_u.q0 = cload(&tsrc->q0);
      tr_u.err = cload(&tsrc->err);
      tr_u.cz_err = cload(&tsrc->cz_err);
      tr_u.errz = cload(&tsrc->errz);
      if constexpr (GK) {
        tr_u.sx = cload(&tsrc->sx); tr_u.sy = cload(&tsrc->sy); tr_u.sz = cload(&tsrc->sz); tr_u.s0 = cload(&tsrc->s0);
      }
      mr = &mr_u;
      if (mine) {
        fp = box_footprint<ROT, GK>(a, &mr_u, &tr_u, bx * 8, bx * 8 + 7, by * 8, by * 8 + 7, bz * tk, bz * tk + tk - 1);
      }
    } else {
      if (mine) fp = box_footprint<ROT, GK>(a, mr, a.tile_maps + m, bx * 8, bx * 8 + 7, by * 8, by * 8 + 7, bz * tk, bz * tk + tk - 1);
    }
    const bool query = mine && (fp.query || fp.partial);
    uint8_t cls = fp.cls;
    const int li = query ? query_level<kQueryTiles>(P, max(fp.x1 - fp.x0, fp.y1 - fp.y0) + 1) : 0x7fff;
    bool from_window = false;
    {
      float2 *__restrict__ win_mm = window_mm[wave * views_per_wave + lane / children];
      uint8_t *__restrict__ win_fl = window_fl[wave * views_per_wave + lane / children];
      int li_w = li;
      for (int off = children >> 1; off > 0; off >>= 1) li_w = min(li_w, __shfl_xor(li_w, off, 64));
      if (li_w != 0x7fff) {
        const int L = kPyramidMinLevel + li_w;
        const bool at_level = query && li == li_w;
        int tx0 = at_level ? fp.x0 >> L : 0x7fffffff, ty0 = at_level ? fp.y0 >> L : 0x7fffffff;
        int tx1 = at_level ? fp.x1 >> L : -1, ty1 = at_level ? fp.y1 >> L : -1;
        int wx0 = tx0, wy0 = ty0, wx1 = tx1, wy1 = ty1;
        for (int off = children >> 1; off > 0; off >>= 1) {
          wx0 = min(wx0, __shfl_xor(wx0, off, 64));
          wy0 = min(wy0, __shfl_xor(wy0, off, 64));
          wx1 = max(wx1, __shfl_xor(wx1, off, 64));
          wy1 = max(wy1, __shfl_xor(wy1, off, 64));
        }
        if (wx1 - wx0 < kWindow && wy1 - wy0 < kWindow) {
          const DepthTile *__restrict__ level = mr->pyramid + P.offset[li_w];
          const int pitch = P.width[li_w];
          const int ww = wx1 - wx0 + 1, wh = wy1 - wy0 + 1;
          const int tx = child & 15;
          for (int ty = child >> 4; ty < wh; ty += children / 16)
            if (tx < ww) {
              const DepthTile t = level[(wy0 + ty) * pitch + wx0 + tx];
              win_mm[ty * kWindow + tx] = make_float2(t.dmin, t.dmax);
              win_fl[ty * kWindow + tx] = (uint8_t)t.flags;
            }
          __builtin_amdgcn_fence(__ATOMIC_RELEASE, "wavefront");
          __builtin_amdgcn_wave_barrier();
          __builtin_amdgcn_fence(__ATOMIC_ACQUIRE, "wavefront");
          if (at_level) {
            TileAcc d;
            for (int ty = ty0; ty <= ty1; ++ty)
              for (int tx = tx0; tx <= tx1; ++tx) {
                const int w = (ty - wy0) * kWindow + (tx - wx0);
                const float2 mm = win_mm[w];
                d.add_tile(DepthTile{mm.x, mm.y, (uint32_t)win_fl[w], 0u});
              }
            cls = fp.partial ? border_class<GK>(a, fp, d) : class_from_bounds(a, d, fp.czmin, fp.czmax);
            from_window = true;
          }
          __builtin_amdgcn_fence(__ATOMIC_RELEASE, "wavefront");
          __builtin_amdgcn_wave_barrier();
        }
      }
    }
    if (query && !from_window) {
      const TileAcc d = pyramid_query<kQueryTiles>(mr->pyramid, P, fp.x0, fp.x1, fp.y0, fp.y1);
      cls = fp.partial ? border_class<GK>(a, fp, d) : class_from_bounds(a, d, fp.czmin, fp.czmax);
    }
    if (mine) out[m] = cls;
  }
}

constexpr int kOriginViews = 8;
constexpr uint32_t kNotWanted = 0xfffffffeu;
template <bool ROT>
__global__ __launch_bounds__(256) void window_origin_kernel(const TileArgs a, const MapRec *__restrict__ maps, int tk,
                                                            uint8_t *__restrict__ classes, WinPair *__restrict__ origins,
                                                            int group_views) {
  __shared__ WinPair tile[kOriginViews][256 + 1];
  __shared__ int64_t rows[256];
  const int bz_first = 2 * a.sbz_first;
  const int bz_count = min(2 * a.super_z, a.bricks_z - bz_first);
  const int64_t n_bricks = (int64_t)a.wbricks_x * a.wbricks_y * bz_count;
  const int lane = threadIdx.x & 63;
  const int64_t local = (int64_t)blockIdx.x * 256 + threadIdx.x;
  const bool exists = local < n_bricks;
  const int bx = (int)(local % a.wbricks_x);
  const int64_t t = local / a.wbricks_x;
  const int by = (int)(t % a.wbricks_y), bz = (int)(t / a.wbricks_y) + bz_first;
  const int64_t row = (((int64_t)bz * a.wbricks_y + by) * a.wbricks_x + bx) * a.class_pitch;
  const bool eligible = exists && bz * tk + tk <= a.nz;
  (void)lane;
  double wxa, wya, wza;
  {
    const double gx = a.ox + (bx * 8 + 0.5) * a.sx;
    const double gy = a.oy + (by * 8 + 0.5) * a.sy;
    const double gz = a.oz + ((bz * tk + a.kz0) + 0.5) * a.sz;
    wxa = row4(a.g + 0, gx, gy, gz), wya = row4(a.g + 4, gx, gy, gz), wza = row4(a.g + 8, gx, gy, gz);
  }
  const int m_begin = a.first_map, m_end = a.first_map + a.n_maps;
  const int g_lo = (m_begin & ~3) + blockIdx.y * group_views;
  rows[threadIdx.x] = row;
  uint32_t held[kOriginViews / 4];
#pragma unroll
  for (int g = 0; g < kOriginViews / 4; ++g) {
    const int m4 = g_lo + 4 * g;
    held[g] = (eligible && 4 * g < group_views && m4 < m_end) ? *reinterpret_cast<const uint32_t *>(classes + row + m4) : 0u;
#pragma unroll
    for (int q = 0; q < 4; ++q) tile[4 * g + q][threadIdx.x].origin = kNotWanted;
  }
#pragma unroll
  for (int g = 0; g < kOriginViews / 4; ++g) {
    const int m4 = g_lo + 4 * g;
    if (4 * g >= group_views || m4 >= m_end) break;
    const uint32_t c4 = held[g];
#pragma unroll 1
    for (int q = 0; q < 4; ++q) {
      const int m = m4 + q;
      const uint8_t c = (uint8_t)(c4 >> (8 * q));
      const bool want = eligible && m >= m_begin && m < m_end && (c & 0x1f) == (uint8_t)(BRICK_MIXED | (MIXED_FREE_OR_NODEPTH << 2));
      if (__builtin_amdgcn_ballot_w64(want) == 0) continue;
      WinPair wp;
      wp.origin = kNotWanted;
      wp.ax = wp.ay = wp.acz = 0.f;
      if (cload(&a.win_recs[m].e_abs) < __builtin_inff()) {
        const MapRec *src = maps + m;
        const TileMapRec *tsrc = a.tile_maps + m;
        const FootRec *fr = a.foot_recs + m;
        const float(*scp)[4] = tk == 16 ? fr->s16 : fr->s8;
        if (want) {
          const double cza = ((cload(&src->rt[8]) * wxa + cload(&src->rt[9]) * wya) + cload(&src->rt[10]) * wza) + cload(&src->rt[11]);
          const double hxa = __builtin_fma(cload(&tsrc->cpx), wxa, __builtin_fma(cload(&tsrc->cpy), wya, __builtin_fma(cload(&tsrc->cpz), wza, cload(&tsrc->cp0))));
          const double hya = __builtin_fma(cload(&tsrc->cqx), wxa, __builtin_fma(cload(&tsrc->cqy), wya, __builtin_fma(cload(&tsrc->cqz), wza, cload(&tsrc->cq0))));
          const float hx0 = (float)hxa, hy0 = (float)hya, z0 = (float)cza;
          float umin = __builtin_inff(), umax = -__builtin_inff(), vmin = __builtin_inff(), vmax = -__builtin_inff();
          float zmin = __builtin_inff(), zmax = -__builtin_inff();
#pragma unroll
          for (int cnr = 0; cnr < 8; ++cnr) {
            const float z = z0 + cload(&scp[cnr][2]);
            const float r = __builtin_amdgcn_rcpf(z);
            const float u = (hx0 + cload(&scp[cnr][0])) * r, v = (hy0 + cload(&scp[cnr][1])) * r;
            umin = __builtin_fminf(umin, u), umax = __builtin_fmaxf(umax, u);
            vmin = __builtin_fminf(vmin, v), vmax = __builtin_fmaxf(vmax, v);
            zmin = __builtin_fminf(zmin, z), zmax = __builtin_fmaxf(zmax, z);
          }
          const float umag = __builtin_fmaxf(__builtin_fmaxf(__builtin_fabsf(umin), __builtin_fabsf(umax)), __builtin_fmaxf(__builtin_fabsf(vmin), __builtin_fabsf(vmax)));
          const float e = 2.0f * cload(&fr->ferr) * __builtin_amdgcn_rcpf(zmin) * (1.0f + 0x1p-20f) + (0x1p-19f * umag + 0x1p-12f);
          const bool sane = zmin > 0.0f && zmax <= (float)(kWinCzRatio * (1.0 - 0x1p-20)) * zmin && umin > -65536.0f && umax < 65536.0f &&
                            vmin > -65536.0f && vmax < 65536.0f && e < 0.25f;
          if (sane) {
            const int cxc = a.W / 2, cyc = a.H / 2;
            const int x0 = (int)__builtin_ceilf(umin - 0.5f - e) + cxc, x1 = (int)__builtin_floorf(umax + 0.5f + e) + cxc;
            const int y0 = (int)__builtin_ceilf(vmin - 0.5f - e) + cyc, y1 = (int)__builtin_floorf(vmax + 0.5f + e) + cyc;
            if (x0 >= -kValidMargin && y0 >= -kValidMargin && x1 < a.W + kValidMargin && y1 < a.H + kValidMargin &&
                x1 - x0 < kWindowCols && y1 - y0 < kWindowRows) {
              wp.origin = (uint32_t)(x0 + kValidMargin) | ((uint32_t)(y0 + kValidMargin) << 16);
              wp.ax = (float)(hxa - (double)(x0 - cxc) * cza);
              wp.ay = (float)(hya - (double)(y0 - cyc) * cza);
              wp.acz = z0;
            }
          }
        }
      }
      if (want) {
        if (wp.origin != kNotWanted)
          tile[4 * g + q][threadIdx.x] = wp;
        else
          classes[row + m] = (uint8_t)(c | CLASS_NO_WINDOW);
      }
    }
  }
  __syncthreads();
  const int v = threadIdx.x & (kOriginViews - 1);
  const int m = g_lo + v;
  if (v < group_views && m < m_end) {
#pragma unroll
    for (int it = 0; it < 8; ++it) {
      const int b = (threadIdx.x >> 3) + 32 * it;
      const WinPair wp = tile[v][b];
      if (wp.origin != kNotWanted) origins[rows[b] + m] = wp;
    }
  }
}


__device__ __forceinline__ bool slot_to_brick(const TileArgs &a, int slot, int &bx, int &by, int &bz) {
  const int within = slot & 31;
  const int code = a.sb_perm[(slot - a.slot_base) >> 5];
  const int sbx = code & 1023, sby = (code >> 10) & 1023, sbz = (code >> 20) + a.sbz_first;
  bx = sbx * 4 + (within & 3);
  by = sby * 4 + ((within >> 2) & 3);
  bz = sbz * 2 + (within >> 4);
  return bx < a.bricks_x && by < a.bricks_y && bz < a.bricks_z;
}

constexpr int kWorkLevels = 4;

__global__ __launch_bounds__(256) void brick_work_kernel(const TileArgs a, int wx, int wy, int n_slots,
                                                         uint8_t *__restrict__ level) {
  const int lane = threadIdx.x & 63;
  const int slot = blockIdx.x * 4 + (threadIdx.x >> 6);
  if (slot >= n_slots) return;
  int bx, by, bz;
  if (!slot_to_brick(a, slot + a.slot_base, bx, by, bz)) {
    if (lane == 0) level[slot] = 255;
    return;
  }
  int mixed = 0, total = 0;
  for (int v = 0; v < wy; ++v)
    for (int u = 0; u < wx; ++u) {
      const int wbx = bx * wx + u, wby = by * wy + v;
      if (wbx >= a.wbricks_x || wby >= a.wbricks_y) continue;
      const uint8_t *row = a.classes + (((int64_t)bz * a.wbricks_y + wby) * a.wbricks_x + wbx) * (int64_t)a.class_pitch;
      for (int m = a.first_map + lane; m < a.first_map + a.n_maps; m += 64) mixed += (row[m] & 3) == BRICK_MIXED ? 1 : 0;
      total += a.n_maps;
    }
  for (int off = 32; off > 0; off >>= 1) mixed += __shfl_xor(mixed, off, 64);
  if (lane == 0) level[slot] = mixed * 2 >= total ? 0 : (mixed * 4 >= total ? 1 : (mixed * 16 >= total ? 2 : 3));
}

constexpr int kOrderChunk = 1024;

__global__ __launch_bounds__(kOrderChunk) void order_count_kernel(const uint8_t *__restrict__ level, int n_slots,
                                                                  int *__restrict__ counts) {
  const int s = blockIdx.x * kOrderChunk + threadIdx.x;
  const int l = s < n_slots ? level[s] : 255;
  for (int q = 0; q < kWorkLevels; ++q) {
    const int c = __syncthreads_count(l == q);
    if (threadIdx.x == 0) counts[blockIdx.x * kWorkLevels + q] = c;
  }
}

__global__ __launch_bounds__(1024) void order_base_kernel(int *__restrict__ counts, int n_chunks, int *__restrict__ n_valid) {
  __shared__ int wave_totals[16];
  __shared__ int carry;
  if (threadIdx.x == 0) carry = 0;
  __syncthreads();
  const int lane = threadIdx.x & 63, wave = threadIdx.x >> 6;
  for (int q = 0; q < kWorkLevels; ++q)
    for (int c0 = 0; c0 < n_chunks; c0 += 1024) {
      const int c = c0 + threadIdx.x;
      const int v = c < n_chunks ? counts[c * kWorkLevels + q] : 0;
      int incl = v;
      for (int off = 1; off < 64; off <<= 1) {
        const int up = __shfl_up(incl, off, 64);
        if (lane >= off) incl += up;
      }
      if (lane == 63) wave_totals[wave] = incl;
      __syncthreads();
      int before = carry, all = 0;
      for (int w = 0; w < 16; ++w) {
        if (w < wave) before += wave_totals[w];
        all += wave_totals[w];
      }
      if (c < n_chunks) counts[c * kWorkLevels + q] = before + incl - v;
      __syncthreads();
      if (threadIdx.x == 0) carry += all;
      __syncthreads();
    }
  if (threadIdx.x == 0) *n_valid = carry;
}

__global__ __launch_bounds__(kOrderChunk) void order_scatter_kernel(const TileArgs a, const uint8_t *__restrict__ level,
                                                                    int n_slots, const int *__restrict__ bases,
                                                                    int *__restrict__ order) {
  __shared__ unsigned long long wave_totals[16];
  const int s = blockIdx.x * kOrderChunk + threadIdx.x;
  const int l = s < n_slots ? level[s] : 255;
  const unsigned long long one = l < kWorkLevels ? 1ull << (16 * l) : 0ull;
  const int lane = threadIdx.x & 63, wave = threadIdx.x >> 6;
  unsigned long long incl = one;
  for (int off = 1; off < 64; off <<= 1) {
    const unsigned long long up = __shfl_up(incl, off, 64);
    if (lane >= off) incl += up;
  }
  if (lane == 63) wave_totals[wave] = incl;
  __syncthreads();
  unsigned long long before = 0;
  for (int w = 0; w < wave; ++w) before += wave_totals[w];
  if (l < kWorkLevels) {
    const int rank = (int)(((before + incl - one) >> (16 * l)) & 0xffffull);
    int bx = 0, by = 0, bz = 0;
    slot_to_brick(a, s + a.slot_base, bx, by, bz);
    order[bases[blockIdx.x * kWorkLevels + l] + rank] = pack_brick(bx, by, bz);
  }
}

constexpr int kOrderOneLaunchSlots = 1 << 18;
__global__ __launch_bounds__(kOrderChunk) void order_rank_kernel(const TileArgs a, const uint8_t *__restrict__ level, int n_slots,
                                                                 int *__restrict__ level_starts, int *__restrict__ order,
                                                                 int *__restrict__ n_valid) {
  __shared__ int partial[16][2 * kWorkLevels];
  __shared__ unsigned long long wave_totals[16];
  const int lane = threadIdx.x & 63, wave = threadIdx.x >> 6;
  int cnt[2 * kWorkLevels];
#pragma unroll
  for (int q = 0; q < 2 * kWorkLevels; ++q) cnt[q] = 0;
  const int pieces = n_slots >> 4;
  const int my_first = blockIdx.x * (kOrderChunk / 16);
  for (int p = threadIdx.x; p < pieces; p += kOrderChunk) {
    const uint4 w = reinterpret_cast<const uint4 *>(level)[p];
    const uint32_t words[4] = {w.x, w.y, w.z, w.w};
    int n[kWorkLevels] = {0, 0, 0, 0};
#pragma unroll
    for (int q = 0; q < 4; ++q) {
      const uint32_t c = words[q];
      const uint32_t ok = (~c >> 7) & 0x01010101u;
      const uint32_t b0 = c & ok, b1 = (c >> 1) & ok;
      const int n3 = __builtin_popcount(b0 & b1), n2 = __builtin_popcount(b1 & ~b0), n1 = __builtin_popcount(b0 & ~b1);
      n[3] += n3, n[2] += n2, n[1] += n1, n[0] += __builtin_popcount(ok) - n1 - n2 - n3;
    }
    const bool before = p < my_first;
#pragma unroll
    for (int l = 0; l < kWorkLevels; ++l) {
      cnt[kWorkLevels + l] += n[l];
      cnt[l] += before ? n[l] : 0;
    }
  }
#pragma unroll
  for (int q = 0; q < 2 * kWorkLevels; ++q) {
    int v = cnt[q];
// ... 31 lines not shown
#pragma unroll
    for (int q = 0; q < kWorkLevels; ++q) base += q < l ? tot[kWorkLevels + q] : (q == l ? tot[q] : 0);
    int bx = 0, by = 0, bz = 0;
    slot_to_brick(a, s + a.slot_base, bx, by, bz);
    order[base + rank] = pack_brick(bx, by, bz);
  }
}

__global__ __launch_bounds__(256) void brick_work_kernel_1x1(const TileArgs a, int n_slots, uint8_t *__restrict__ level) {
  const int lane = threadIdx.x & 63;
  const int slot = (blockIdx.x * 4 + (threadIdx.x >> 6)) * 4 + (lane >> 4);
  const int part = lane & 15;
  int bx = 0, by = 0, bz = 0;
  const bool exists = slot < n_slots;
  const bool in_grid = exists && slot_to_brick(a, slot + a.slot_base, bx, by, bz);
  int mixed = 0, light = 0;
  constexpr uint32_t kLight = (uint32_t)BRICK_MIXED | ((uint32_t)MIXED_FREE_OR_NODEPTH << 2);
  static_assert(BRICK_MIXED == 0, "a mixed pair's low two bits are 00");
  if (in_grid) {
    const uint8_t *row = a.classes + (((int64_t)bz * a.wbricks_y + by) * a.wbricks_x + bx) * (int64_t)a.class_pitch + a.first_map;
    for (int v0 = part * 16; v0 < a.n_maps; v0 += 256) {
      if (((a.first_map | a.class_pitch) & 15) == 0 && v0 + 16 <= a.n_maps) {
        const uint4 w = *reinterpret_cast<const uint4 *>(row + v0);
        const uint32_t words[4] = {w.x, w.y, w.z, w.w};
#pragma unroll
        for (int q = 0; q < 4; ++q) {
          const uint32_t c = words[q];
          const uint32_t nz = (c | (c >> 1)) & 0x01010101u;
          mixed += 4 - __builtin_popcount(nz);
          const uint32_t y = (c & 0x3f3f3f3fu) ^ (kLight * 0x01010101u);
          light += 4 - __builtin_popcount((y + 0x7f7f7f7fu) & 0x80808080u);
        }
      } else {
        for (int v = v0; v < min(v0 + 16, a.n_maps); ++v) {
          mixed += (row[v] & 3) == BRICK_MIXED ? 1 : 0;
          light += (row[v] & 0x3f) == kLight ? 1 : 0;
        }
      }
    }
  }
  for (int off = 8; off > 0; off >>= 1) {
    mixed += __shfl_xor(mixed, off, 64);
    light += __shfl_xor(light, off, 64);
  }
  if (a.flags & TILE_FLAG_COST_ORDER) {
    const int lv = !in_grid ? 255 : (mixed == 0 ? kCostLevels - 1 : (kCostLevels - 1) - (mixed * (kCostLevels - 1) + a.n_maps - 1) / a.n_maps);
    if (exists && part == 0) level[slot] = (uint8_t)lv;
    unsigned long long todo = __builtin_amdgcn_ballot_w64(exists && part == 0 && lv < kCostLevels);
    while (todo) {
      const int l0 = __shfl(lv, __builtin_ctzll(todo), 64);
      const unsigned long long same = __builtin_amdgcn_ballot_w64(lv == l0) & todo;
      if (lane == __builtin_ctzll(todo)) atomicAdd(const_cast<int32_t *>(a.order_levels) + l0, __builtin_popcountll(same));
      todo &= ~same;
    }
    return;
  }
  if (exists && part == 0)
    {
      const int cost2 = a.win_origin ? 2 * light + 5 * (mixed - light) : 2 * mixed;
      level[slot] = !in_grid ? 255 : (cost2 >= a.n_maps ? 0 : (cost2 * 2 >= a.n_maps ? 1 : (cost2 * 8 >= a.n_maps ? 2 : 3)));
    }
}

__global__ __launch_bounds__(kOrderChunk) void order_cost_kernel(const TileArgs a, const uint8_t *__restrict__ level, int n_slots,
                                                                 int *__restrict__ order, int *__restrict__ n_valid) {
  __shared__ int base[kCostLevels];
  int32_t *sizes = const_cast<int32_t *>(a.order_levels), *cursors = sizes + kCostLevels;
  const int lane = threadIdx.x & 63;
  if (threadIdx.x < 64) {
    const int v = sizes[lane];
    int incl = v;
    for (int off = 1; off < 64; off <<= 1) {
      const int up = __shfl_up(incl, off, 64);
      if (lane >= off) incl += up;
    }
    base[lane] = incl - v;
    if (blockIdx.x == 0 && lane == 63) *n_valid = incl;
  }
  __syncthreads();
  const int s = blockIdx.x * kOrderChunk + threadIdx.x;
  const int lv = s < n_slots ? level[s] : 255;
  int pos = -1;
  unsigned long long todo = __builtin_amdgcn_ballot_w64(lv < kCostLevels);
  while (todo) {
    const int leader = __builtin_ctzll(todo);
    const int l0 = __shfl(lv, leader, 64);
    const unsigned long long same = __builtin_amdgcn_ballot_w64(lv == l0) & todo;
    int first = 0;
    if (lane == leader) first = atomicAdd(cursors + l0, __builtin_popcountll(same));
    first = __shfl(first, leader, 64);
    if (lv == l0) pos = base[l0] + first + __builtin_popcountll(same & ((1ull << lane) - 1ull));
    todo &= ~same;
  }
  if (pos >= 0) {
    int bx = 0, by = 0, bz = 0;
    slot_to_brick(a, s + a.slot_base, bx, by, bz);
    order[pos] = pack_brick(bx, by, bz);
  }
}

inline unsigned blocks_of(int64_t n) { return (unsigned)((n + 255) / 256); }

}

PyramidDesc make_pyramid_desc(int W, int H) {
  PyramidDesc P;
  std::memset(&P, 0, sizeof(P));
  int off = 0;
  for (int li = 0; li < kPyramidMaxLevels; ++li) {
    const int L = kPyramidMinLevel + li, S = 1 << L;
    P.width[li] = (W + S - 1) / S;
    P.height[li] = (H + S - 1) / S;
    P.offset[li] = off;
    off += P.width[li] * P.height[li];
    P.n_levels = li + 1;
    if (P.width[li] == 1 && P.height[li] == 1) break;
  }
  P.total_tiles = off;
  return P;
}

hipError_t launch_upload_views(const void *in, int in_is_f64, const double *best_cost, double threshold, void *out, int out_is_f64,
                               int64_t n_maps, int W, int H, const PyramidDesc &P, DepthTile *pyramids, uint8_t *valid, uint32_t *bits,
                               unsigned long long *counters, hipStream_t stream) {
  if (n_maps <= 0) return hipSuccess;
  if (n_maps > 65535) return hipErrorInvalidConfiguration;
  const int cover_x = std::max(W + 2 * kValidMargin, valid_bits_tiles_x(W) * 32);
  const int cover_y = std::max(((H + 2 * kValidMargin + 7) / 8) * 8, valid_bits_tiles_y(H) * 32);
  const dim3 grid((unsigned)((cover_x + 511) / 512), (unsigned)((cover_y + 7) / 8), (unsigned)n_maps);
#define DMI_UPLOAD(IN, OUT)                                                                                                      \
  hipLaunchKernelGGL((upload_views_kernel<IN, OUT>), grid, dim3(512), 0, stream, static_cast<const IN *>(in), best_cost, threshold, \
                     static_cast<OUT *>(out), W, H, P, pyramids, valid, bits, counters)
  if (in_is_f64) {
    if (out_is_f64)
      DMI_UPLOAD(double, double);
    else
      DMI_UPLOAD(double, float);
  } else {
    if (out_is_f64)
      DMI_UPLOAD(float, double);
    else
      DMI_UPLOAD(float, float);
  }
#undef DMI_UPLOAD
  return hipGetLastError();
}

hipError_t launch_build_pyramid_levels(int64_t n_maps, const PyramidDesc &P, DepthTile *pyramids, hipStream_t stream) {
  if (n_maps <= 0 || P.n_levels <= 1) return hipSuccess;
  hipLaunchKernelGGL(pyramid_levels_kernel, dim3((unsigned)n_maps), dim3(1024), 0, stream, P, pyramids);
  return hipGetLastError();
}

hipError_t launch_window_origins(const TileArgs &a, const MapRec *maps_dev, int tk, uint8_t *classes, int general_k,
                                 hipStream_t stream) {
  if (general_k || !a.win_origin || a.n_maps <= 0) return hipSuccess;
  const int bz_count = std::min(2 * a.super_z, a.bricks_z - 2 * a.sbz_first);
  const int64_t n_bricks = (int64_t)a.wbricks_x * a.wbricks_y * bz_count;
  if (n_bricks <= 0) return hipSuccess;
  const int64_t brick_groups = (n_bricks + 255) / 256;
  const int span = a.first_map + a.n_maps - (a.first_map & ~3);
  int group_views = kOriginViews;
  while (group_views > 4 && brick_groups * ((span + group_views - 1) / group_views) < 2048) group_views >>= 1;
  const dim3 grid((unsigned)brick_groups, (unsigned)((span + group_views - 1) / group_views));
  if (a.rotated)
    hipLaunchKernelGGL((window_origin_kernel<true>), grid, dim3(256), 0, stream, a, maps_dev, tk, classes, a.win_origin, group_views);
  else
    hipLaunchKernelGGL((window_origin_kernel<false>), grid, dim3(256), 0, stream, a, maps_dev, tk, classes, a.win_origin, group_views);
  return hipGetLastError();
}

hipError_t launch_classify_bricks(const TileArgs &a, const MapRec *maps_dev, const PyramidDesc &P, int tk, uint8_t *classes,
                                  uint8_t *coarse, int general_k, hipStream_t stream) {
  const int bz_count = std::min(2 * a.super_z, a.bricks_z - 2 * a.sbz_first);
  const int64_t n_bricks = (int64_t)a.wbricks_x * a.wbricks_y * bz_count;
  if (n_bricks <= 0 || a.n_maps <= 0) return hipSuccess;
  if (n_bricks > (int64_t)0x7fffffff || (a.n_maps + 3) / 4 > 65535) return hipErrorInvalidConfiguration;
  const int per_z = 32 / tk;
  const int64_t n_boxes = (int64_t)((a.wbricks_x + 3) / 4) * ((a.wbricks_y + 3) / 4) * ((bz_count + per_z - 1) / per_z);
  const dim3 coarse_grid((unsigned)((n_boxes + 3) / 4), (unsigned)((a.n_maps + 63) / 64));
#define DMI_LAUNCH_COARSE(R, G) \
  hipLaunchKernelGGL((classify_coarse_kernel<R, G>), coarse_grid, dim3(64, 4), 0, stream, a, maps_dev, P, tk, classes, coarse)
  if (a.rotated && general_k)
    DMI_LAUNCH_COARSE(true, true);
  else if (a.rotated)
    DMI_LAUNCH_COARSE(true, false);
  else if (general_k)
    DMI_LAUNCH_COARSE(false, true);
  else
    DMI_LAUNCH_COARSE(false, false);
#undef DMI_LAUNCH_COARSE
  hipError_t e = hipGetLastError();
  if (e != hipSuccess) return e;
  int group_views = 64;
  while (group_views > 8 && n_boxes * ((a.n_maps + group_views - 1) / group_views) < 2048) group_views >>= 1;
  const dim3 fine_grid((unsigned)n_boxes, (unsigned)((a.n_maps + group_views - 1) / group_views));
  [[maybe_unused]] int q = 5;
#ifdef DMI_TUNING
  if (const char *env = getenv("DMI_QUERY_TILES")) q = atoi(env);
#endif
  const bool wide = tk == 8;
#define DMI_LAUNCH_FINE_G(Q, C, R, G) \
  hipLaunchKernelGGL((classify_kernel<Q, C, R, G>), fine_grid, dim3(256), 0, stream, a, maps_dev, P, tk, classes, coarse, group_views)
#define DMI_LAUNCH_FINE_R(Q, C, R)      \
  do {                                  \
    if (general_k)                      \
      DMI_LAUNCH_FINE_G(Q, C, R, true); \
    else                                \
      DMI_LAUNCH_FINE_G(Q, C, R, false);\
  } while (0)
#define DMI_LAUNCH_FINE(Q)                      \
  do {                                          \
    if (wide && a.rotated)                      \
      DMI_LAUNCH_FINE_R(Q, 64, true);           \
    else if (wide)                              \
      DMI_LAUNCH_FINE_R(Q, 64, false);          \
    else if (a.rotated)                         \
      DMI_LAUNCH_FINE_R(Q, 32, true);           \
    else                                        \
      DMI_LAUNCH_FINE_R(Q, 32, false);          \
  } while (0)
#ifdef DMI_TUNING
  if (q <= 2)
    DMI_LAUNCH_FINE(2);
  else if (q == 3)
    DMI_LAUNCH_FINE(3);
  else
#endif
    DMI_LAUNCH_FINE(5);
#undef DMI_LAUNCH_FINE_G
#undef DMI_LAUNCH_FINE_R
#undef DMI_LAUNCH_FINE
  return hipGetLastError();
}

int64_t coarse_class_bytes(const TileArgs &a, int tk) {
  const int per_z = 32 / tk;
  return (int64_t)((a.wbricks_x + 3) / 4) * ((a.wbricks_y + 3) / 4) * ((a.bricks_z + per_z - 1) / per_z) * (int64_t)a.class_pitch;
}

hipError_t launch_order_bricks(const TileArgs &a, int wx, int wy, uint8_t *level, int *order, int *n_valid,
                               hipStream_t stream) {
  const int n_slots = a.super_x * a.super_y * a.super_z * 32;
  if (wx == 1 && wy == 1)
    hipLaunchKernelGGL(brick_work_kernel_1x1, dim3((unsigned)((n_slots + 15) / 16)), dim3(256), 0, stream, a, n_slots, level);
  else
    hipLaunchKernelGGL(brick_work_kernel, dim3((unsigned)((n_slots + 3) / 4)), dim3(256), 0, stream, a, wx, wy, n_slots, level);
  hipError_t e = hipGetLastError();
  if (e != hipSuccess) return e;
  int *counts = reinterpret_cast<int *>(level + ((size_t)n_slots + 15) / 16 * 16);
  const int n_chunks = (n_slots + kOrderChunk - 1) / kOrderChunk;
  if ((a.flags & TILE_FLAG_COST_ORDER) && wx == 1 && wy == 1) {
    hipLaunchKernelGGL(order_cost_kernel, dim3((unsigned)n_chunks), dim3(kOrderChunk), 0, stream, a, level, n_slots, order, n_valid);
    return hipGetLastError();
  }
  if (n_slots <= kOrderOneLaunchSlots) {
    hipLaunchKernelGGL(order_rank_kernel, dim3((unsigned)n_chunks), dim3(kOrderChunk), 0, stream, a, level, n_slots, counts, order, n_valid);
    return hipGetLastError();
  }
  hipLaunchKernelGGL(order_count_kernel, dim3((unsigned)n_chunks), dim3(kOrderChunk), 0, stream, level, n_slots, counts);
  hipLaunchKernelGGL(order_base_kernel, dim3(1), dim3(1024), 0, stream, counts, n_chunks, n_valid);
  hipLaunchKernelGGL(order_scatter_kernel, dim3((unsigned)n_chunks), dim3(kOrderChunk), 0, stream, a, level, n_slots, counts, order);
  return hipGetLastError();
}

size_t order_scratch_bytes(size_t n_slots) {
  return (n_slots + 15) / 16 * 16 + std::max<size_t>(((n_slots + kOrderChunk - 1) / kOrderChunk) * kWorkLevels, 2 * kCostLevels) * sizeof(int) + 64;
}

}
```

cudadepthmapintegration_amd/csrc/fusion_kernels.h:

```cpp
#pragma once

#include <hip/hip_runtime.h>
#include <stddef.h>
#include <stdint.h>
#include <string.h>

struct dmi_context;

namespace dmi {

int grid_pointer_for_sums(::dmi_context *ctx, void **ptr);

struct alignas(16) DepthTile {
  float dmin, dmax;
  uint32_t flags;
  uint32_t pad;
};
enum TileFlags : uint32_t { TILE_HAS_SENTINEL = 1, TILE_HAS_VALID = 2, TILE_HAS_NAN = 4, TILE_PART_HOLE_FREE = 8, TILE_PART_NO_VALID = 16 };
constexpr int64_t kNoClassesMaxBricks = 1024;
constexpr int kNoClassesMaxViews = 48;
constexpr uint8_t COARSE_CHILDREN_WRITTEN = 0x80;

constexpr int kPyramidMinLevel = 3;
constexpr int kPyramidMaxLevels = 13;
// ... 4 lines not shown
  int32_t width[kPyramidMaxLevels];
  int32_t height[kPyramidMaxLevels];
  int32_t offset[kPyramidMaxLevels];
};

struct alignas(16) MapRec {
  double rt[12];
  double k[12];
  const void *depth;
  const DepthTile *pyramid;
};
static_assert(sizeof(MapRec) == 208, "MapRec layout");

struct alignas(16) TileMapRec {
  double rz0, rz1, rz3;
  double px, py, pz, p0;
  double qx, qy, qz, q0;
  double dhx, dhy;
  double err;
  const void *depth;
  double cz_err;
  double errk;
  double sx, sy, sz, s0, dhz, errz;
  double cpx, cpy, cpz, cp0, cqx, cqy, cqz, cq0;
  double cdhx, cdhy, cerrk;
  float t1_dhx, t1_dhy, t1_dcz, t1_dthr;
  float t1_e1, t1_c1;
  float t1_erel, t1_hspan;
  int32_t t1_cidx;
  int32_t t1_ok;
  const uint8_t *valid;
  float vm_c0, vm_w8;
  int32_t vm_base, vm_bytes;
  const uint32_t *vbits;
  int32_t vb_bytes;
  int32_t vb_rowskip;
  int32_t vb_mx, vb_my;
  float t1_b;
  int32_t vb_pad;
};
#ifndef DMI_TIER1
#define DMI_TIER1 1
#endif
constexpr int kValidMargin = 32;
constexpr unsigned kValidByte = 10;
__host__ __device__ inline int64_t valid_map_bytes(int W, int H) {
  return (int64_t)((H + 2 * kValidMargin + 7) / 8) * (W + 2 * kValidMargin) * 8;
}
__host__ __device__ inline int valid_bits_tiles_x(int W) { return (W + 2 * kValidMargin + 31) / 32 + 1; }
__host__ __device__ inline int valid_bits_tiles_y(int H) { return (H + 2 * kValidMargin + 31) / 32; }
__host__ __device__ inline int64_t valid_bits_bytes(int W, int H) { return (int64_t)valid_bits_tiles_x(W) * valid_bits_tiles_y(H) * 128; }
constexpr int kWindowCols = 32, kWindowRows = 64;
constexpr uint8_t CLASS_NO_WINDOW = 0x20;
static_assert(sizeof(TileMapRec) == 368, "TileMapRec layout");

struct alignas(64) WinRec {
  const uint32_t *vbits;
  float di[2], dj[2], dk[2];
  float ci[2], cj[2], ck[2];
  float e_abs;
  float c1;
};
static_assert(sizeof(WinRec) == 64, "WinRec is one cache line");
struct alignas(64) FootRec {
  float s8[8][4];
  float s16[8][4];
  float ferr, pad[15];
};
static_assert(sizeof(FootRec) == 320, "FootRec layout");
constexpr float kWinC1 = 0.5f - 0x1p-14f;
constexpr double kWinCzRatio = 1.25;
struct alignas(16) WinPair {
  uint32_t origin;
  float ax, ay, acz;
};
static_assert(sizeof(WinPair) == 16, "WinPair layout");

enum KMode : int {
  K_GENERAL = 0,
  K_PINHOLE_SKEW = 1,
  K_PINHOLE = 2
};

struct FuseArgs {
  int32_t nx, ny, nz;
  int32_t W, H;
  int32_t first_map, n_maps;
  int32_t init_from_grid;
  int32_t kz0, pad1;
  int32_t k_first, k_count;
  double ox, oy, oz;
  double sx, sy, sz;
  double g[12];
  double thick, delta;
  double rho_pos, rho_neg, rho_zero;
  double slope;
  double free_space;
  const MapRec *maps;
  void *grid;
  uint32_t *voxel_hits;
  unsigned long long *map_hits;
};

struct TileArgs {
  int32_t nx, ny, nz, W, H, first_map, n_maps, init_from_grid;
  int32_t kpad;
  int32_t bricks_x, bricks_y, bricks_z;
  int32_t super_x, super_y, super_z;
  int32_t sbz_first, pad3;
  int32_t slot_base, slot_count;
  int32_t depth_bytes;
  int32_t kz0, pad1;
  double ox, oy, oz, sx, sy, sz;
  double g[12];
  double thick, delta, rho_pos, rho_neg, slope, free_space;
  const TileMapRec *tile_maps;
  const double *cz_table;
  void *grid;
  uint32_t *voxel_hits;
  unsigned long long *map_hits;
  const FuseArgs *full;
  const uint8_t *classes;
  int32_t class_pitch;
  int32_t wbricks_x, wbricks_y;
  int32_t xcd_run_wg;
  const int32_t *order;
  const int32_t *n_order;
  unsigned long long behind_mask;
  int32_t rotated;
  int32_t flags;
  const MapRec *maps;
  const int32_t *order_levels;
  const double *free_sums;
  const int32_t *sb_perm;
  unsigned long long *wg_times;
  int64_t wg_times_n;
  int32_t *queue_heads;
  WinPair *win_origin;
  int64_t win_delta;
  const WinRec *win_recs;
  const FootRec *foot_recs;
  int32_t vb_bytes, vb_rowskip;
  int32_t win_cx, win_cy;
};
constexpr int kFreeSumsMax = 4096;
__host__ __device__ inline int32_t pack_brick(int bx, int by, int bz) { return (int32_t)((uint32_t)bx | ((uint32_t)by << 11) | ((uint32_t)bz << 22)); }
static_assert(offsetof(TileArgs, nx) == 0 && offsetof(TileArgs, nz) == 8 && offsetof(TileArgs, kpad) == 32 &&
                  offsetof(TileArgs, bricks_x) == 36 && offsetof(TileArgs, bricks_z) == 44 && offsetof(TileArgs, sbz_first) == 60,
              "TileArgs head layout");
enum TileKernelFlags : int32_t {
  TILE_FLAG_NO_INTERIOR = 1,
  TILE_FLAG_XCD_RUNS = 2,
  TILE_FLAG_COST_ORDER = 4,
  TILE_FLAG_DBG_SKIP_WINDOW_PAIRS = 256,
  TILE_FLAG_DBG_ONLY_WINDOW_PAIRS = 512,
  TILE_FLAG_DBG_NO_WINDOW_LOADS = 1024
};

enum BrickClass : uint8_t {
  BRICK_MIXED = 0,
  BRICK_FREE = 1,
  BRICK_BEHIND = 2,
  BRICK_SKIP = 3
};

enum MixedReason : uint8_t {
  MIXED_UNSPECIFIED = 0,
  MIXED_DEGENERATE = 1,
  MIXED_CAMERA_PLANE = 2,
  MIXED_IMAGE_BORDER = 3,
  MIXED_NAN_DEPTH = 4,
  MIXED_SENTINEL_AND_DEPTH = 5,
  MIXED_NEAR_SURFACE = 6,
  MIXED_FREE_OR_NODEPTH = 7
};

struct FuseConfig {
  int depth_is_f64;
  int grid_is_f64;
  int k_mode;
  int count_hits;
  int variant;
  int use_tile;
  int general_k;
  int holes;
};

enum VariantBits : int {
  VAR_EXACT_DIVISION = 1,
  VAR_GENERAL_K = 2,
  VAR_BLOCK_SHAPE_MASK = 12,
  VAR_FORCE_GENERAL = 16,
  VAR_TILE_SHAPE_MASK = 0xE0,
  VAR_TILE_SHAPE_SHIFT = 5,
  VAR_NO_BRICK_CLASSES = 256,
  VAR_SPATIAL_ORDER = 512,
  VAR_FIXED_TILE_SHAPE = 4096,
  VAR_KEEP_BEHIND_ADDS = 1024,
  VAR_NO_INTERIOR = 2048,
  VAR_XCD_RUNS = 8192,
  VAR_ZMAJOR_SLOTS = 16384,
  VAR_PERSISTENT_ALWAYS = 32768,
  VAR_PERSISTENT_NEVER = 65536,
  VAR_BRICK_CLASSES_ALWAYS = 131072,
  VAR_NO_WINDOWS = 262144,
  VAR_WINDOWS_ALWAYS = 524288,
  VAR_COST_ORDER = 1048576,
  VAR_NO_COST_ORDER = 2097152
};

constexpr int kMaxColumnHeight = 16;
struct TileShape {
  int tk, wx, wy;
};
TileShape tile_shape(int variant, bool depth_is_f64, bool rotated, bool general_k);

hipError_t launch_fuse(const FuseArgs &args, const FuseConfig &cfg, hipStream_t stream);

hipError_t launch_fuse_tiled(const TileArgs &args, const MapRec *maps_dev, const FuseConfig &cfg, const PyramidDesc &pyramid,
                             uint8_t *order_scratch, uint8_t *coarse_classes, hipEvent_t before_main_kernel,
                             hipStream_t stream);

hipError_t launch_widen_depth(const float *in, double *out, int64_t n, hipStream_t stream);
hipError_t launch_convert_grid(const void *in, int in_is_f64, void *out, int64_t n, hipStream_t stream);

hipError_t launch_fp64_probe(double *out, int blocks, int iters, hipStream_t stream);

PyramidDesc make_pyramid_desc(int W, int H);
hipError_t launch_upload_views(const void *in, int in_is_f64, const double *best_cost, double threshold, void *out, int out_is_f64,
                               int64_t n_maps, int W, int H, const PyramidDesc &desc, DepthTile *pyramids, uint8_t *valid, uint32_t *bits,
                               unsigned long long *counters, hipStream_t stream);
hipError_t launch_build_pyramid_levels(int64_t n_maps, const PyramidDesc &desc, DepthTile *pyramids, hipStream_t stream);
hipError_t launch_window_origins(const TileArgs &args, const MapRec *maps_dev, int tk, uint8_t *classes, int general_k,
                                 hipStream_t stream);
hipError_t launch_classify_bricks(const TileArgs &args, const MapRec *maps_dev, const PyramidDesc &desc, int tk,
                                  uint8_t *classes, uint8_t *coarse, int general_k, hipStream_t stream);
int64_t coarse_class_bytes(const TileArgs &args, int tk);
constexpr int kCostOrderMaxSlots = 0;
size_t order_scratch_bytes(size_t n_slots);
hipError_t launch_order_bricks(const TileArgs &args, int wx, int wy, uint8_t *level, int *order, int *n_valid,
                               hipStream_t stream);

hipError_t launch_cell_to_point(const void *cells, int cells_are_f64, double *points, int nx, int ny, int nz,
                                hipStream_t stream);

size_t iso_block_count(int nx, int ny, int nz);
hipError_t launch_iso_count(const double *points, int nx, int ny, int nz, double iso, uint32_t *counts, uint64_t *bases,
                            void *scan_temp, size_t *scan_temp_bytes, hipStream_t stream);
hipError_t launch_iso_write(const double *points, int nx, int ny, int nz, double iso, const uint64_t *bases, int64_t *ids,
                            uint64_t capacity, hipStream_t stream);

struct MeshGeom {
  int nx, ny, nz, segs_per_row;
  double iso;
  double origin[3], spacing[3];
  double m[12];
  uint64_t n_vertices, n_triangles;
};
struct MeshNormals {
  double nm[9];
  float *normals;
};
int isosurface_max_triangles_per_cell();
size_t isosurface_segment_count(int nx, int ny, int nz);
hipError_t launch_isosurface_count(const double *points, const MeshGeom &g, uint32_t *counts, uint64_t *bases, void *scan_temp,
                                   size_t *scan_temp_bytes, hipStream_t stream);
hipError_t launch_isosurface_write(const double *points, const MeshGeom &g, const uint64_t *bases, double *verts, int64_t *tris,
                                   const MeshNormals *normals, hipStream_t stream);

struct ComponentsMesh {
  uint64_t n_vertices, n_triangles;
  const double *vertices;
  const float *normals;
  const int64_t *triangles;
  double *out_vertices;
  float *out_normals;
  int64_t *out_triangles;
  int64_t *region_id;
  int64_t *region_size;
};
struct ComponentsScratch {
  uint32_t *parent, *size;
  uint32_t *vmap, *rmap;
  uint32_t *tmap;
  unsigned long long *counters;
  void *scan_temp;
  size_t scan_temp_bytes;
};
hipError_t components_scan_temp_bytes(uint64_t n_vertices, uint64_t n_triangles, size_t *bytes);
hipError_t launch_isosurface_components(const ComponentsMesh &m, const ComponentsScratch &s, int largest, uint64_t min_triangles,
                                        hipEvent_t *events, hipStream_t stream);

struct SmoothMesh {
  uint64_t n_vertices, n_triangles;
  const double *vertices;
  const int64_t *triangles;
  float *normals_out;
};
struct SmoothScratch {
  uint64_t *keys[2];
  uint32_t *row_start;
  uint32_t *valence, *offsets;
  unsigned long long *fixed;
  double *positions[2];
  void *temp;
  size_t temp_bytes;
};
hipError_t smooth_temp_bytes(uint64_t n_vertices, uint64_t n_triangles, size_t *bytes);
hipError_t launch_isosurface_smooth(const SmoothMesh &m, const SmoothScratch &s, int iterations, double lambda, double mu,
                                    double **result, hipEvent_t *events, hipStream_t stream);

}
```

cudadepthmapintegration_amd/csrc/fusion_tile.hip:

```cpp
#include <stdlib.h>

#include <algorithm>
#include <type_traits>

#include "fusion_kernels.h"
#include "fusion_device.h"

#ifndef DMI_T1_CHAINS
#define DMI_T1_CHAINS 4
#endif
#ifndef DMI_T1_COLUMN_CHAINS
#define DMI_T1_COLUMN_CHAINS 2
#endif
#if !defined(DMI_TUNING) && (defined(DMI_EXP_SKIP_WINDOW_VIEWS) || defined(DMI_EXP_SAME_REC) || defined(DMI_EXP_NO_WINDOW_LOADS) || \
                             defined(DMI_EXP_NO_LANE_MARGIN))
#error "a DMI_EXP_* switch that changes results was defined without DMI_TUNING"
#endif

namespace dmi {

int tile_shape_index(int variant);

namespace {

// ... 1144 lines not shown

template <typename DepthT, typename GridT, int TK, int WX, int WY, int MINW, int GROUP, bool ROT = false, bool GENK = false, bool WIN = false>
hipError_t launch_shape(const TileArgs &a, const FuseConfig &cfg, hipStream_t s) {
  static_assert(TK <= kMaxColumnHeight, "dmi_multi_z_slab aligns slabs to kMaxColumnHeight");
  constexpr bool one_wave = WX * WY == 1;
  constexpr bool rare = std::is_same<DepthT, double>::value || GENK;
  static_assert(!WIN || (one_wave && !rare), "window launches are production launches");
  const int per_round = 8 * a.xcd_run_wg;
  unsigned blocks = (unsigned)((a.super_x * a.super_y * a.super_z * 32 + 32 + per_round - 1) / per_round * per_round);
  const dim3 block(64 * WX * WY);
  const bool zf = a.behind_mask != 0 && !cfg.count_hits;
  if (WIN && !zf) return hipErrorInvalidValue;
  bool stay = true;
  if constexpr (one_wave && !rare) {
    const int64_t voxels = (int64_t)a.super_x * a.super_y * a.super_z * 32 * 64 * TK;
    stay = (cfg.variant & VAR_PERSISTENT_ALWAYS) ? true
           : (cfg.variant & VAR_PERSISTENT_NEVER) ? false
           : (cfg.variant & VAR_NO_BRICK_CLASSES) ? true
           : cfg.holes ? (a.n_maps >= 48 && voxels >= (int64_t(1) << 25))
                       : (a.n_maps >= kPersistentMinViews && voxels >= (int64_t(1) << 27));
  }
  auto launch = [&](auto kernel, bool persistent) {
    unsigned n = blocks;
    if (persistent && one_wave) {
      static const unsigned resident = resident_workgroups(kernel, 64);
      n = std::min(n, resident);
    }
    hipLaunchKernelGGL(kernel, dim3(n), block, 0, s, a);
    return hipGetLastError();
  };
  if constexpr (!WIN) {
    if (cfg.count_hits) return launch(fuse_tile_kernel<DepthT, GridT, TK, WX, WY, MINW, GROUP, true, ROT, GENK>, true);
  }
  if constexpr (one_wave && !rare) {
    if (zf) {
      if (!stay) return launch(fuse_tile_kernel<DepthT, GridT, TK, WX, WY, MINW, GROUP, false, ROT, GENK, false, WIN, true>, false);
      return launch(fuse_tile_kernel<DepthT, GridT, TK, WX, WY, MINW, GROUP, false, ROT, GENK, true, WIN, true>, true);
    }
  }
  if constexpr (!WIN) return launch(fuse_tile_kernel<DepthT, GridT, TK, WX, WY, MINW, GROUP, false, ROT, GENK>, true);
  return hipErrorInvalidValue;
}

int effective_shape(int variant, bool depth_is_f64, bool rotated, bool general_k = false) {
  int shape = tile_shape_index(variant);
#ifndef DMI_TUNING
  shape = (shape == 1 || shape == 3 || shape == 4 || shape == 7) ? 7 : 0;
#endif
  if (general_k || depth_is_f64) return 0;
  return (rotated && shape != 7) ? 0 : shape;
}

template <typename DepthT, typename GridT, int TK, int MINW, bool ROT>
hipError_t launch_win(const TileArgs &a, const FuseConfig &cfg, hipStream_t s) {
  if constexpr (DMI_TIER1 != 0 && std::is_same<DepthT, float>::value)
    return launch_shape<DepthT, GridT, TK, 1, 1, MINW, 8, ROT, false, true>(a, cfg, s);
  else
    return hipErrorInvalidValue;
}

template <typename DepthT, typename GridT>
hipError_t launch_types(const TileArgs &a, const FuseConfig &cfg, hipStream_t s) {
  constexpr bool f32_depth = std::is_same<DepthT, float>::value;
  const int shape = effective_shape(cfg.variant, !f32_depth, a.rotated != 0, cfg.general_k != 0);
  const bool win = DMI_TIER1 != 0 && std::is_same<DepthT, float>::value && a.win_origin != nullptr && !cfg.count_hits && !cfg.general_k &&
                   a.behind_mask != 0;
#ifdef DMI_FAST_BUILD
  if (win) {
    if (shape == 7) return launch_win<DepthT, GridT, 8, 6, false>(a, cfg, s);
    return launch_win<DepthT, GridT, 16, 5, false>(a, cfg, s);
  }
  if constexpr (f32_depth) {
    if (shape == 7) return launch_shape<DepthT, GridT, 8, 1, 1, 6, 8>(a, cfg, s);
  }
  return launch_shape<DepthT, GridT, 16, 1, 1, 5, 8>(a, cfg, s);
#else
  if (cfg.general_k) {
    if (a.rotated) return launch_shape<DepthT, GridT, 16, 1, 1, 5, 8, true, true>(a, cfg, s);
    return launch_shape<DepthT, GridT, 16, 1, 1, 5, 8, false, true>(a, cfg, s);
  }
  if (a.rotated) {
    if (win) {
      if (shape == 7) return launch_win<DepthT, GridT, 8, 6, true>(a, cfg, s);
      return launch_win<DepthT, GridT, 16, 5, true>(a, cfg, s);
    }
    if constexpr (f32_depth) {
      if (shape == 7) return launch_shape<DepthT, GridT, 8, 1, 1, 6, 8, true>(a, cfg, s);
    }
    return launch_shape<DepthT, GridT, 16, 1, 1, 5, 8, true>(a, cfg, s);
  }
#ifdef DMI_TUNING
  if constexpr (std::is_same<DepthT, float>::value) {
    switch (shape) {
      case 1: return launch_shape<DepthT, GridT, 8, 2, 2, 6, 8>(a, cfg, s);
      case 2: return launch_shape<DepthT, GridT, 16, 2, 2, 5, 8>(a, cfg, s);
      case 3: return launch_shape<DepthT, GridT, 8, 2, 2, 6, 4>(a, cfg, s);
      case 4: return launch_shape<DepthT, GridT, 8, 2, 2, 7, 8>(a, cfg, s);
      case 5: return launch_shape<DepthT, GridT, 16, 2, 2, 5, 4>(a, cfg, s);
      case 6: return launch_shape<DepthT, GridT, 16, 2, 2, 6, 2>(a, cfg, s);
      default: break;
    }
  }
#endif
  if (win && (shape == 7 || shape == 0)) {
    if (shape == 7) return launch_win<DepthT, GridT, 8, 6, false>(a, cfg, s);
    return launch_win<DepthT, GridT, 16, 5, false>(a, cfg, s);
  }
  if constexpr (f32_depth) {
    if (shape == 7) return launch_shape<DepthT, GridT, 8, 1, 1, 6, 8>(a, cfg, s);
  }
  return launch_shape<DepthT, GridT, 16, 1, 1, 5, 8>(a, cfg, s);
#endif
}

}

int tile_shape_index(int variant) { return (variant & VAR_TILE_SHAPE_MASK) >> VAR_TILE_SHAPE_SHIFT; }

TileShape tile_shape(int variant, bool depth_is_f64, bool rotated, bool general_k) {
  switch (effective_shape(variant, depth_is_f64, rotated, general_k)) {
    case 0: return TileShape{16, 1, 1};
    case 7: return TileShape{8, 1, 1};
    case 1:
    case 3:
    case 4: return TileShape{8, 2, 2};
    default: return TileShape{16, 2, 2};
  }
}

#ifdef DMI_TUNING
__global__ __launch_bounds__(256) void remap_classes_kernel(uint8_t *classes, int64_t n, uint32_t table) {
  for (int64_t i = (int64_t)blockIdx.x * blockDim.x + threadIdx.x; i < n; i += (int64_t)gridDim.x * blockDim.x) {
    const uint8_t b = classes[i];
    classes[i] = (uint8_t)((table >> (8 * (b & 3))) & 0xff);
  }
}
#endif

hipError_t launch_fuse_tiled(const TileArgs &a, const MapRec *maps_dev, const FuseConfig &cfg, const PyramidDesc &pyramid,
                             uint8_t *order_scratch, uint8_t *coarse_classes, hipEvent_t before_main_kernel,
                             hipStream_t stream) {
  if (a.n_maps <= 0) return hipSuccess;
  hipError_t e = hipSuccess;
  if (cfg.variant & VAR_NO_BRICK_CLASSES) {
    const int64_t entries = a.rotated ? a.kpad : (int64_t)a.kpad * a.n_maps;
    hipLaunchKernelGGL(launch_tables_kernel, dim3((unsigned)std::min<int64_t>((entries + 255) / 256, 4096)), dim3(256), 0, stream, a, maps_dev);
    e = hipGetLastError();
    if (e != hipSuccess) return e;
  }
  if (!(cfg.variant & VAR_NO_BRICK_CLASSES)) {
    const TileShape sh = tile_shape(cfg.variant, cfg.depth_is_f64 != 0, a.rotated != 0, cfg.general_k != 0);
    e = launch_classify_bricks(a, maps_dev, pyramid, sh.tk, const_cast<uint8_t *>(a.classes), coarse_classes, cfg.general_k, stream);
    if (e != hipSuccess) return e;
    e = launch_window_origins(a, maps_dev, sh.tk, const_cast<uint8_t *>(a.classes), cfg.general_k, stream);
    if (e != hipSuccess) return e;
#ifdef DMI_TUNING
    if (const char *env = getenv("DMI_DEBUG_CLASS_REMAP")) {
      const int64_t n = (int64_t)a.wbricks_x * a.wbricks_y * a.bricks_z * (int64_t)a.class_pitch;
      hipLaunchKernelGGL(remap_classes_kernel, dim3(4096), dim3(256), 0, stream, const_cast<uint8_t *>(a.classes), n,
                         (uint32_t)strtoul(env, nullptr, 0));
    }
#endif
    if (a.order) {
      e = launch_order_bricks(a, sh.wx, sh.wy, order_scratch, const_cast<int *>(a.order), const_cast<int *>(a.n_order), stream);
      if (e != hipSuccess) return e;
    }
  }
  if (before_main_kernel) {
    e = hipEventRecord(before_main_kernel, stream);
    if (e != hipSuccess) return e;
  }
#ifndef DMI_FAST_BUILD
  if (cfg.depth_is_f64) {
    if (cfg.grid_is_f64) return launch_types<double, double>(a, cfg, stream);
    return launch_types<double, float>(a, cfg, stream);
  }
  if (cfg.grid_is_f64) return launch_types<float, double>(a, cfg, stream);
#endif
  return launch_types<float, float>(a, cfg, stream);
}

}
```

include/dmi.h:

```cpp
#ifndef DMI_H_
#define DMI_H_

#include <stddef.h>
#include <stdint.h>

#ifdef __cplusplus
extern "C" {
#endif

#define DMI_ABI_VERSION 5

typedef struct dmi_context dmi_context;

typedef enum dmi_status {
  DMI_OK = 0,
  DMI_ERR_INVALID_ARGUMENT = 1,
  DMI_ERR_DEVICE = 2,
  DMI_ERR_OUT_OF_MEMORY = 3,
  DMI_ERR_STATE = 4
} dmi_status;

typedef enum dmi_dtype { DMI_F32 = 0, DMI_F64 = 1 } dmi_dtype;

typedef enum dmi_depth_storage { DMI_DEPTH_AUTO = 0, DMI_DEPTH_F32 = 1, DMI_DEPTH_F64 = 2 } dmi_depth_storage;

typedef struct dmi_grid_desc {
  int32_t cell_dims[3];
  double origin[3];
  double spacing[3];
  double grid_matrix[16];
} dmi_grid_desc;

typedef struct dmi_ray_potential {
  double thickness;
  double rho;
  double eta;
  double delta;
} dmi_ray_potential;

typedef struct dmi_options {
  int32_t device;
  int32_t grid_dtype;
  int32_t depth_storage;
  int32_t count_hits;
  int32_t kernel_variant;
  int32_t z_first;
  void *stream;
  void *external_grid;
} dmi_options;

typedef struct dmi_timings {
  double last_fuse_kernel_ms;
  double total_fuse_kernel_ms;
  uint64_t fuse_launches;
  double last_upload_ms;
  double last_download_ms;
  double last_cell_to_point_ms;
  double last_fuse_main_kernel_ms;
  double total_fuse_main_kernel_ms;
} dmi_timings;

typedef struct dmi_info {
  int64_t n_voxels;
  int32_t n_views;
  int32_t depth_width;
  int32_t depth_height;
  int32_t depth_storage_in_use;
  int32_t grid_dtype;
  int32_t k_mode;
  int32_t kernel_variant;
  int32_t tiled_kernel;
  uint64_t device_bytes;
  uint64_t pixels_without_depth;
} dmi_info;

void dmi_default_options(dmi_options *opt);

int dmi_create(const dmi_grid_desc *grid, const dmi_ray_potential *ray, const dmi_options *opt, dmi_context **out);

void dmi_destroy(dmi_context *ctx);

const char *dmi_last_error(const dmi_context *ctx);

int dmi_add_views(dmi_context *ctx, const double *depth, const double *best_cost, double threshold, const double *K4,
                  const double *RT4, int32_t n, int32_t width, int32_t height);

int dmi_add_views_f32(dmi_context *ctx, const float *depth, const double *K4, const double *RT4, int32_t n,
                      int32_t width, int32_t height);

int dmi_clear_views(dmi_context *ctx);

int dmi_reset_grid(dmi_context *ctx);

int dmi_upload_grid(dmi_context *ctx, const double *grid);

int dmi_fuse(dmi_context *ctx);

int dmi_fuse_range(dmi_context *ctx, int32_t first, int32_t count);

#define DMI_SLAB_ALIGNMENT 32
int dmi_fuse_slab(dmi_context *ctx, int32_t z_first, int32_t z_count);

int dmi_synchronize(dmi_context *ctx);

int dmi_download_grid_f64(dmi_context *ctx, double *out);
int dmi_download_grid_f32(dmi_context *ctx, float *out);

int dmi_fuse_range_download(dmi_context *ctx, int32_t first, int32_t count, void *out, int32_t out_dtype, int32_t n_slabs);

int dmi_download_hits(dmi_context *ctx, uint32_t *voxel_hits, uint64_t *map_hits);

int dmi_grid_device_pointer(dmi_context *ctx, void **ptr);

int dmi_cell_to_point(dmi_context *ctx);
int dmi_download_point_data_f64(dmi_context *ctx, double *out);
int dmi_point_data_device_pointer(dmi_context *ctx, void **ptr);

int dmi_iso_active_cells(dmi_context *ctx, double iso, uint64_t *count, int64_t *cell_ids, uint64_t capacity);

int dmi_extract_isosurface(dmi_context *ctx, double iso, uint64_t *n_vertices, uint64_t *n_triangles);
int dmi_download_isosurface(dmi_context *ctx, double *vertices, int64_t *triangles);
int dmi_extract_isosurface_normals(dmi_context *ctx, double iso, uint64_t *n_vertices, uint64_t *n_triangles);
int dmi_download_isosurface_normals(dmi_context *ctx, float *normals);
int dmi_get_isosurface_kernel_ms(dmi_context *ctx, double *last);

enum { DMI_COMPONENTS_MIN_TRIANGLES = 0, DMI_COMPONENTS_LARGEST = 1 };
int dmi_filter_isosurface_components(dmi_context *ctx, int mode, uint64_t min_triangles, uint64_t *n_vertices, uint64_t *n_triangles,
                                     uint64_t *n_components, uint64_t *n_components_kept);
int dmi_download_isosurface_regions(dmi_context *ctx, int64_t *region_id, int64_t *region_size);
int dmi_get_isosurface_filter_kernel_ms(dmi_context *ctx, double *last);
int dmi_get_isosurface_filter_pass_ms(dmi_context *ctx, double out[4]);
int dmi_get_isosurface_filter_cas_retries(dmi_context *ctx, uint64_t *last);

int dmi_smooth_isosurface(dmi_context *ctx, int32_t iterations, double lambda, double mu);
int dmi_get_isosurface_smooth_kernel_ms(dmi_context *ctx, double *last);
int dmi_get_isosurface_smooth_pass_ms(dmi_context *ctx, double out[3]);

int dmi_get_brick_class_histogram(dmi_context *ctx, uint64_t out[4]);

int dmi_get_mixed_reason_histogram(dmi_context *ctx, uint64_t out[8]);

int dmi_get_window_pair_count(dmi_context *ctx, uint64_t *out);

int dmi_get_view_paths(dmi_context *ctx, uint64_t out[6]);

int dmi_get_timings(dmi_context *ctx, dmi_timings *out);
int dmi_get_info(dmi_context *ctx, dmi_info *out);
size_t dmi_sizeof_info(void);
size_t dmi_sizeof_timings(void);

int dmi_get_upload_kernel_ms(dmi_context *ctx, double *last, double *total);

int dmi_alloc_pinned(size_t bytes, void **out);
int dmi_free_pinned(void *ptr);
int dmi_pcie_probe(int32_t device, size_t bytes, double *h2d_GBps, double *d2h_GBps);
int dmi_fp64_probe(int32_t device, double milliseconds, double *tflops);

int dmi_color_mesh(const double *points, int64_t n_points, const uint8_t *colors, const double *K4, const double *RT4,
                   int32_t n_views, int32_t width, int32_t height, int32_t device, uint8_t *mean, uint8_t *median,
                   int32_t *count);
const char *dmi_color_last_error(void);

typedef struct dmi_color_context dmi_color_context;
int dmi_color_create(int32_t device, dmi_color_context **out);
void dmi_color_destroy(dmi_color_context *ctx);
int dmi_color_add_views(dmi_color_context *ctx, const uint8_t *colors, const double *K4, const double *RT4, int32_t n,
                        int32_t width, int32_t height);
int dmi_color_clear_views(dmi_color_context *ctx);
int dmi_color_process(dmi_color_context *ctx, const double *points, int64_t n_points, uint8_t *mean, uint8_t *median,
                      int32_t *count);
int dmi_color_set_scratch_budget(dmi_color_context *ctx, uint64_t bytes);
int dmi_color_set_vertex_reorder(dmi_color_context *ctx, int32_t enable);
int dmi_color_get_kernel_ms(dmi_color_context *ctx, double *out);
int dmi_color_add_views_with_depth(dmi_color_context *ctx, const uint8_t *colors, const double *depths, const double *K4,
                                   const double *RT4, int32_t n, int32_t width, int32_t height);
int dmi_color_set_depth_test(dmi_color_context *ctx, int32_t enable, double tolerance);

typedef struct dmi_multi_context dmi_multi_context;

typedef enum dmi_partition { DMI_PARTITION_VIEWS = 0, DMI_PARTITION_Z_SLABS = 1 } dmi_partition;
typedef enum dmi_exchange { DMI_EXCHANGE_ALL_REDUCE = 0, DMI_EXCHANGE_REDUCE_SCATTER = 1, DMI_EXCHANGE_PEER_COPY = 2 } dmi_exchange;

#define DMI_UNIQUE_ID_BYTES 128

typedef struct dmi_multi_options {
  int32_t grid_dtype;
  int32_t depth_storage;
  int32_t kernel_variant;
  int32_t partition;
  int32_t exchange;
  int32_t n_slabs;
} dmi_multi_options;

typedef struct dmi_multi_info {
  int32_t world;
  int32_t n_local;
  int32_t first_rank;
  int32_t rccl_ranks;
  int32_t rccl_version;
  int32_t partition, exchange, n_slabs;
  int64_t n_voxels;
  int64_t n_views_total;
  int64_t n_views_local;
} dmi_multi_info;

typedef struct dmi_multi_timings {
  double last_step_ms;
  double last_fuse_kernel_ms;
  double total_step_ms;
  uint64_t steps;
} dmi_multi_timings;

void dmi_multi_default_options(dmi_multi_options *opt);

int dmi_multi_view_shard(int64_t n, int32_t rank, int32_t world, int64_t *first, int64_t *count);
#define DMI_Z_SLAB_ALIGNMENT 16
int dmi_multi_z_slab(int32_t nz, int32_t rank, int32_t world, int32_t *z_first, int32_t *z_count);
int dmi_multi_peer_chunk(int64_t n, int32_t world, int32_t c, int64_t *first, int64_t *count);
int dmi_multi_slab_ranges(int32_t nz, int32_t n_slabs, int32_t *z_first, int32_t *z_count, int32_t max_slabs);

int dmi_multi_create(const dmi_grid_desc *grid, const dmi_ray_potential *ray, const dmi_multi_options *opt,
                     const int32_t *devices, int32_t n, dmi_multi_context **out);
int dmi_multi_get_unique_id(uint8_t id[DMI_UNIQUE_ID_BYTES]);
int dmi_multi_create_rank(const dmi_grid_desc *grid, const dmi_ray_potential *ray, const dmi_multi_options *opt,
                          int32_t device, int32_t rank, int32_t world, const uint8_t id[DMI_UNIQUE_ID_BYTES],
                          dmi_multi_context **out);
void dmi_multi_destroy(dmi_multi_context *ctx);
const char *dmi_multi_last_error(const dmi_multi_context *ctx);

int dmi_multi_add_views(dmi_multi_context *ctx, const double *depth, const double *best_cost, double threshold,
                        const double *K4, const double *RT4, int32_t n, int32_t width, int32_t height);
int dmi_multi_add_views_f32(dmi_multi_context *ctx, const float *depth, const double *K4, const double *RT4, int32_t n,
                            int32_t width, int32_t height);
int dmi_multi_add_local_views(dmi_multi_context *ctx, int32_t local_index, const double *depth, const double *best_cost,
                              double threshold, const double *K4, const double *RT4, int32_t n, int32_t width, int32_t height);
int dmi_multi_add_local_views_f32(dmi_multi_context *ctx, int32_t local_index, const float *depth, const double *K4,
                                  const double *RT4, int32_t n, int32_t width, int32_t height);
int dmi_multi_clear_views(dmi_multi_context *ctx);

int dmi_multi_fuse(dmi_multi_context *ctx);
int dmi_multi_synchronize(dmi_multi_context *ctx);

int dmi_multi_download_grid_f32(dmi_multi_context *ctx, float *out, int64_t *owned_first, int64_t *owned_count);
int dmi_multi_download_grid_f64(dmi_multi_context *ctx, double *out, int64_t *owned_first, int64_t *owned_count);

int dmi_multi_get_info(dmi_multi_context *ctx, dmi_multi_info *out);
int dmi_multi_get_timings(dmi_multi_context *ctx, dmi_multi_timings *out);
int dmi_multi_local_context(dmi_multi_context *ctx, int32_t local_index, dmi_context **out);

int dmi_abi_version(void);
int dmi_device_count(void);

#ifdef __cplusplus
}
#endif

#endif
```

Measured before the change: 2910.

## Compute window origins inside classify kernel, leave only residual origin pass

Moves per-pair window-origin computation into the fine classify kernel for non-general-k paths, using wave-uniform readlane and ballot iteration over views. The separate window_origin kernel now runs only in residual mode, driven by coarse-class marks and exiting early for blocks without work. It also adds waves_per_eu attributes on classify_kernel and a debug API that dumps pair tables. The aim is to avoid re-reading classes and recomputing brick anchors in a second pass, at the cost of more register pressure and serialized per-view work in the classify kernel.

```diff
diff --git a/cudadepthmapintegration_amd/capi.py b/cudadepthmapintegration_amd/capi.py
--- a/cudadepthmapintegration_amd/capi.py
+++ b/cudadepthmapintegration_amd/capi.py
@@ -29,6 +29,7 @@
 VARIANT_WINDOWS_ALWAYS = 524288
 VARIANT_COST_ORDER = 1048576
 VARIANT_NO_COST_ORDER = 2097152
+VARIANT_ORIGINS_SEPARATE = 4194304
 VARIANT_BRICK_CLASSES_ALWAYS = 131072
 VARIANT_FIXED_TILE_SHAPE = 4096
 VARIANT_SPATIAL_ORDER = 512
@@ -94,7 +95,7 @@
     "dmi_get_brick_class_histogram", "dmi_get_timings", "dmi_get_info", "dmi_alloc_pinned", "dmi_free_pinned", "dmi_pcie_probe", "dmi_fp64_probe", "dmi_abi_version", "dmi_device_count",
     "dmi_color_mesh", "dmi_color_last_error", "dmi_cell_to_point", "dmi_download_point_data_f64",
     "dmi_point_data_device_pointer", "dmi_color_create", "dmi_color_destroy", "dmi_color_add_views",
-    "dmi_color_clear_views", "dmi_color_process", "dmi_color_get_kernel_ms", "dmi_get_mixed_reason_histogram", "dmi_get_window_pair_count", "dmi_get_view_paths", "dmi_get_upload_kernel_ms", "dmi_sizeof_info", "dmi_sizeof_timings",
+    "dmi_color_clear_views", "dmi_color_process", "dmi_color_get_kernel_ms", "dmi_get_mixed_reason_histogram", "dmi_get_window_pair_count", "dmi_get_pair_tables", "dmi_get_view_paths", "dmi_get_upload_kernel_ms", "dmi_sizeof_info", "dmi_sizeof_timings",
     "dmi_color_set_scratch_budget", "dmi_color_set_vertex_reorder", "dmi_color_add_views_with_depth", "dmi_color_set_depth_test",
     "dmi_iso_active_cells",
     "dmi_extract_isosurface", "dmi_download_isosurface", "dmi_get_isosurface_kernel_ms",
@@ -188,6 +189,8 @@
     L.dmi_get_mixed_reason_histogram.argtypes = [vp, ctypes.POINTER(ctypes.c_uint64)]
     if hasattr(L, "dmi_get_window_pair_count"):
         L.dmi_get_window_pair_count.argtypes = [vp, ctypes.POINTER(ctypes.c_uint64)]
+    if hasattr(L, "dmi_get_pair_tables"):
+        L.dmi_get_pair_tables.argtypes = [vp, vp, vp, ctypes.c_int64, ctypes.POINTER(ctypes.c_int64), ctypes.POINTER(ctypes.c_int32)]
     if hasattr(L, "dmi_get_view_paths"):
         L.dmi_get_view_paths.argtypes = [vp, ctypes.POINTER(ctypes.c_uint64)]
     if hasattr(L, "dmi_get_upload_kernel_ms"):
@@ -551,6 +554,16 @@
             return 0
         self._check(self._lib.dmi_get_window_pair_count(self._h, ctypes.byref(n)))
         return int(n.value)
+
+    def pair_tables(self) -> tuple:
+        b, v = ctypes.c_int64(0), ctypes.c_int32(0)
+        self._check(self._lib.dmi_get_pair_tables(self._h, None, None, 0, ctypes.byref(b), ctypes.byref(v)))
+        classes = np.zeros((b.value, v.value), np.uint8)
+        pairs = np.zeros((b.value, v.value, 4), np.uint32)
+        if classes.size:
+            self._check(self._lib.dmi_get_pair_tables(self._h, classes.ctypes.data_as(ctypes.c_void_p), pairs.ctypes.data_as(ctypes.c_void_p),
+                                                      classes.size, ctypes.byref(b), ctypes.byref(v)))
+        return classes, pairs
 
     def upload_kernel_ms(self) -> tuple:
         if not hasattr(self._lib, "dmi_get_upload_kernel_ms"):
diff --git a/cudadepthmapintegration_amd/csrc/dmi_capi.hip b/cudadepthmapintegration_amd/csrc/dmi_capi.hip
--- a/cudadepthmapintegration_amd/csrc/dmi_capi.hip
+++ b/cudadepthmapintegration_amd/csrc/dmi_capi.hip
@@ -1287,7 +1287,8 @@
     t.grid = a.grid; t.voxel_hits = a.voxel_hits; t.map_hits = a.map_hits;
     t.rotated = grid_axis_aligned(ctx->grid) ? 0 : 1;
     t.flags = ((cfg.variant & dmi::VAR_NO_INTERIOR) ? dmi::TILE_FLAG_NO_INTERIOR : 0) |
-              ((cfg.variant & dmi::VAR_XCD_RUNS) ? dmi::TILE_FLAG_XCD_RUNS : 0);
+              ((cfg.variant & dmi::VAR_XCD_RUNS) ? dmi::TILE_FLAG_XCD_RUNS : 0) |
+              ((cfg.variant & dmi::VAR_ORIGINS_SEPARATE) ? dmi::TILE_FLAG_ORIGINS_SEPARATE : 0);
     t.maps = ctx->d_maps;
     const size_t table_doubles = std::max<size_t>((size_t)n_views, 4) * (size_t)t.kpad;
     const size_t need = table_doubles + (size_t)dmi::kFreeSumsMax + 1;
@@ -2264,6 +2265,44 @@
   });
 }
 
+int dmi_get_pair_tables(dmi_context *ctx, uint8_t *classes, void *win_pairs, int64_t capacity_pairs, int64_t *bricks, int32_t *views) {
+  return guarded(ctx, "dmi_get_pair_tables", [&]() -> int {
+  if (!ctx || !bricks || !views) return fail(ctx, DMI_ERR_INVALID_ARGUMENT, "dmi_get_pair_tables: null argument");
+  *bricks = 0;
+  *views = 0;
+  if (!ctx->last_fuse_classes) return DMI_OK;
+  *bricks = ctx->last_class_bricks;
+  *views = ctx->last_count;
+  const int64_t n_bricks = ctx->last_class_bricks;
+  const int64_t n_views = ctx->last_count;
+  if (!classes || capacity_pairs < n_bricks * n_views) return DMI_OK;
+  DMI_HIP(ctx, hipSetDevice(ctx->opt.device));
+  const size_t pairs = (size_t)n_bricks * ctx->last_class_pitch;
+  std::vector<uint8_t> host(pairs);
+  DMI_HIP(ctx, hipMemcpyAsync(host.data(), ctx->d_classes, pairs, hipMemcpyDeviceToHost, ctx->stream));
+  std::vector<dmi::WinPair> entries;
+  if (win_pairs && ctx->last_win_origin) {
+    entries.resize(pairs);
+    DMI_HIP(ctx, hipMemcpyAsync(entries.data(), ctx->last_win_origin, pairs * sizeof(dmi::WinPair), hipMemcpyDeviceToHost, ctx->stream));
+  }
+  DMI_HIP(ctx, hipStreamSynchronize(ctx->stream));
+  if (win_pairs) std::memset(win_pairs, 0, (size_t)(n_bricks * n_views) * sizeof(dmi::WinPair));
+  const int64_t per_layer = n_bricks / std::max<int64_t>(1, ctx->last_bricks_z);
+  for (int64_t b = 0; b < n_bricks; ++b) {
+    const int64_t bz = b / std::max<int64_t>(1, per_layer);
+    const bool top_inside = bz * ctx->last_tk + ctx->last_tk <= ctx->grid.cell_dims[2];
+    const size_t base = (size_t)b * ctx->last_class_pitch + ctx->last_first;
+    for (int64_t m = 0; m < n_views; ++m) {
+      const uint8_t c = host[base + (size_t)m];
+      classes[b * n_views + m] = c;
+      if (!entries.empty() && top_inside && (c & 0x3f) == (dmi::BRICK_MIXED | (dmi::MIXED_FREE_OR_NODEPTH << 2)))
+        std::memcpy(static_cast<uint8_t *>(win_pairs) + (size_t)(b * n_views + m) * sizeof(dmi::WinPair), &entries[base + (size_t)m], sizeof(dmi::WinPair));
+    }
+  }
+  return DMI_OK;
+  });
+}
+
 int dmi_get_timings(dmi_context *ctx, dmi_timings *out) {
   return guarded(ctx, "dmi_get_timings", [&]() -> int {
   if (!ctx || !out) return fail(ctx, DMI_ERR_INVALID_ARGUMENT, "dmi_get_timings: null argument");
diff --git a/cudadepthmapintegration_amd/csrc/fusion_classify.hip b/cudadepthmapintegration_amd/csrc/fusion_classify.hip
--- a/cudadepthmapintegration_amd/csrc/fusion_classify.hip
+++ b/cudadepthmapintegration_amd/csrc/fusion_classify.hip
@@ -402,6 +402,66 @@
   return class_from_bounds(a, pyramid_query<kQueryTiles>(mr->pyramid, P, fp.x0, fp.x1, fp.y0, fp.y1), fp.czmin, fp.czmax);
 }
 
+constexpr uint8_t kWindowClass = (uint8_t)(BRICK_MIXED | (MIXED_FREE_OR_NODEPTH << 2));
+template <bool UNIFORM, typename T>
+__device__ __forceinline__ T rec_load(const T *p) {
+  if constexpr (UNIFORM)
+    return cload(p);
+  else
+    return *p;
+}
+
+template <bool UNIFORM>
+__device__ __forceinline__ bool pair_window(const TileArgs &a, const MapRec *__restrict__ maps, int tk, int m, double wxa, double wya,
+                                            double wza, WinPair &wp) {
+  if (!(rec_load<UNIFORM>(&a.win_recs[m].e_abs) < __builtin_inff())) return false;
+  const MapRec *src = maps + m;
+  const TileMapRec *tsrc = a.tile_maps + m;
+  const FootRec *fr = a.foot_recs + m;
+  const float(*scp)[4] = tk == 16 ? fr->s16 : fr->s8;
+  const double cza = ((rec_load<UNIFORM>(&src->rt[8]) * wxa + rec_load<UNIFORM>(&src->rt[9]) * wya) + rec_load<UNIFORM>(&src->rt[10]) * wza) +
+                     rec_load<UNIFORM>(&src->rt[11]);
+  const double hxa = __builtin_fma(rec_load<UNIFORM>(&tsrc->cpx), wxa, __builtin_fma(rec_load<UNIFORM>(&tsrc->cpy), wya,
+                                   __builtin_fma(rec_load<UNIFORM>(&tsrc->cpz), wza, rec_load<UNIFORM>(&tsrc->cp0))));
+  const double hya = __builtin_fma(rec_load<UNIFORM>(&tsrc->cqx), wxa, __builtin_fma(rec_load<UNIFORM>(&tsrc->cqy), wya,
+                                   __builtin_fma(rec_load<UNIFORM>(&tsrc->cqz), wza, rec_load<UNIFORM>(&tsrc->cq0))));
+  const float hx0 = (float)hxa, hy0 = (float)hya, z0 = (float)cza;
+  float umin = __builtin_inff(), umax = -__builtin_inff(), vmin = __builtin_inff(), vmax = -__builtin_inff();
+  float zmin = __builtin_inff(), zmax = -__builtin_inff();
+#pragma unroll
+  for (int cnr = 0; cnr < 8; ++cnr) {
+    const float z = z0 + rec_load<UNIFORM>(&scp[cnr][2]);
+    const float r = __builtin_amdgcn_rcpf(z);
+    const float u = (hx0 + rec_load<UNIFORM>(&scp[cnr][0])) * r, v = (hy0 + rec_load<UNIFORM>(&scp[cnr][1])) * r;
+    umin = __builtin_fminf(umin, u), umax = __builtin_fmaxf(umax, u);
+    vmin = __builtin_fminf(vmin, v), vmax = __builtin_fmaxf(vmax, v);
+    zmin = __builtin_fminf(zmin, z), zmax = __builtin_fmaxf(zmax, z);
+  }
+  const float umag = __builtin_fmaxf(__builtin_fmaxf(__builtin_fabsf(umin), __builtin_fabsf(umax)), __builtin_fmaxf(__builtin_fabsf(vmin), __builtin_fabsf(vmax)));
+  const float e = 2.0f * rec_load<UNIFORM>(&fr->ferr) * __builtin_amdgcn_rcpf(zmin) * (1.0f + 0x1p-20f) + (0x1p-19f * umag + 0x1p-12f);
+  const bool sane = zmin > 0.0f && zmax <= (float)(kWinCzRatio * (1.0 - 0x1p-20)) * zmin && umin > -65536.0f && umax < 65536.0f &&
+                    vmin > -65536.0f && vmax < 65536.0f && e < 0.25f;
+  if (!sane) return false;
+  const int cxc = a.W / 2, cyc = a.H / 2;
+  const int x0 = (int)__builtin_ceilf(umin - 0.5f - e) + cxc, x1 = (int)__builtin_floorf(umax + 0.5f + e) + cxc;
+  const int y0 = (int)__builtin_ceilf(vmin - 0.5f - e) + cyc, y1 = (int)__builtin_floorf(vmax + 0.5f + e) + cyc;
+  if (!(x0 >= -kValidMargin && y0 >= -kValidMargin && x1 < a.W + kValidMargin && y1 < a.H + kValidMargin && x1 - x0 < kWindowCols &&
+        y1 - y0 < kWindowRows))
+    return false;
+  wp.origin = (uint32_t)(x0 + kValidMargin) | ((uint32_t)(y0 + kValidMargin) << 16);
+  wp.ax = (float)(hxa - (double)(x0 - cxc) * cza);
+  wp.ay = (float)(hya - (double)(y0 - cyc) * cza);
+  wp.acz = z0;
+  return true;
+}
+
+__device__ __forceinline__ void brick_anchor(const TileArgs &a, int tk, int bx, int by, int bz, double &wxa, double &wya, double &wza) {
+  const double gx = a.ox + (bx * 8 + 0.5) * a.sx;
+  const double gy = a.oy + (by * 8 + 0.5) * a.sy;
+  const double gz = a.oz + ((bz * tk + a.kz0) + 0.5) * a.sz;
+  wxa = row4(a.g + 0, gx, gy, gz), wya = row4(a.g + 4, gx, gy, gz), wza = row4(a.g + 8, gx, gy, gz);
+}
+
 constexpr int kCostLevels = 64;
 
 template <bool ROT, bool GK>
@@ -456,9 +516,10 @@
 constexpr int kWindow = 16;
 
 template <int kQueryTiles, int kChildren, bool ROT, bool GK>
-__global__ __launch_bounds__(256) void classify_kernel(const TileArgs a, const MapRec *__restrict__ maps,
+__global__ __launch_bounds__(256) __attribute__((amdgpu_waves_per_eu(GK ? 1 : (ROT ? 4 : 5)))) void classify_kernel(const TileArgs a, const MapRec *__restrict__ maps,
                                                        const PyramidDesc P, int tk, uint8_t *__restrict__ classes,
-                                                       const uint8_t *__restrict__ coarse, int group_views) {
+                                                       const uint8_t *__restrict__ coarse, int group_views,
+                                                       WinPair *__restrict__ origins) {
   constexpr int children = kChildren;
   constexpr int views_per_wave = 64 / children;
   constexpr int per_z = children / 16;
@@ -482,7 +543,7 @@
   const int child = lane % children;
   const int bx = cbx * 4 + (child & 3), by = cby * 4 + ((child >> 2) & 3), bz = cbz * per_z + (child >> 4);
   const bool in_grid = bx < a.wbricks_x && by < a.wbricks_y && bz < bz_first + bz_count;
-  uint8_t *__restrict__ out = classes + (int64_t)((bz * a.wbricks_y + by) * a.wbricks_x + bx) * a.class_pitch;
+  const int64_t row = (int64_t)((bz * a.wbricks_y + by) * a.wbricks_x + bx) * a.class_pitch;
   while (items) {
     const int first = __builtin_ctzll(items);
     items &= items - 1;
@@ -575,22 +636,41 @@
       const TileAcc d = pyramid_query<kQueryTiles>(mr->pyramid, P, fp.x0, fp.x1, fp.y0, fp.y1);
       cls = fp.partial ? border_class<GK>(a, fp, d) : class_from_bounds(a, d, fp.czmin, fp.czmax);
     }
-    if (mine) out[m] = cls;
+    if constexpr (!GK) {
+      if (origins != nullptr) {
+        const bool windowed = mine && bz * tk + tk <= a.nz && (cls & 0x1f) == kWindowClass;
+#pragma unroll 1
+        for (int h = 0; h < views_per_wave; ++h) {
+          const bool now = windowed && lane / children == h;
+          if (__builtin_amdgcn_ballot_w64(now) == 0) continue;
+          const int mh = __builtin_amdgcn_readlane(m, h * children);
+          if (now) {
+            double wxa, wya, wza;
+            brick_anchor(a, tk, bx, by, bz, wxa, wya, wza);
+            WinPair wp;
+            if (pair_window<true>(a, maps, tk, mh, wxa, wya, wza, wp))
+              origins[row + mh] = wp;
+            else
+              cls |= CLASS_NO_WINDOW;
+          }
+        }
+      }
+    }
+    if (mine) classes[row + m] = cls;
   }
 }
 
 constexpr int kOriginViews = 8;
 constexpr uint32_t kNotWanted = 0xfffffffeu;
-template <bool ROT>
+template <bool ROT, bool RESIDUAL>
 __global__ __launch_bounds__(256) void window_origin_kernel(const TileArgs a, const MapRec *__restrict__ maps, int tk,
-                                                            uint8_t *__restrict__ classes, WinPair *__restrict__ origins,
-                                                            int group_views) {
+                                                            uint8_t *__restrict__ classes, const uint8_t *__restrict__ coarse,
+                                                            WinPair *__restrict__ origins, int group_views) {
   __shared__ WinPair tile[kOriginViews][256 + 1];
   __shared__ int64_t rows[256];
   const int bz_first = 2 * a.sbz_first;
   const int bz_count = min(2 * a.super_z, a.bricks_z - bz_first);
   const int64_t n_bricks = (int64_t)a.wbricks_x * a.wbricks_y * bz_count;
-  const int lane = threadIdx.x & 63;
   const int64_t local = (int64_t)blockIdx.x * 256 + threadIdx.x;
   const bool exists = local < n_bricks;
   const int bx = (int)(local % a.wbricks_x);
@@ -598,25 +678,31 @@
   const int by = (int)(t % a.wbricks_y), bz = (int)(t / a.wbricks_y) + bz_first;
   const int64_t row = (((int64_t)bz * a.wbricks_y + by) * a.wbricks_x + bx) * a.class_pitch;
   const bool eligible = exists && bz * tk + tk <= a.nz;
-  (void)lane;
-  double wxa, wya, wza;
-  {
-    const double gx = a.ox + (bx * 8 + 0.5) * a.sx;
-    const double gy = a.oy + (by * 8 + 0.5) * a.sy;
-    const double gz = a.oz + ((bz * tk + a.kz0) + 0.5) * a.sz;
-    wxa = row4(a.g + 0, gx, gy, gz), wya = row4(a.g + 4, gx, gy, gz), wza = row4(a.g + 8, gx, gy, gz);
+  const uint8_t *__restrict__ marks = classes + row;
+  if constexpr (RESIDUAL) {
+    const int per_z = 32 / tk;
+    const int cx_n = (a.wbricks_x + 3) / 4, cy_n = (a.wbricks_y + 3) / 4;
+    marks = coarse + (int64_t)(((bz / per_z) * cy_n + (by >> 2)) * cx_n + (bx >> 2)) * a.class_pitch;
   }
   const int m_begin = a.first_map, m_end = a.first_map + a.n_maps;
   const int g_lo = (m_begin & ~3) + blockIdx.y * group_views;
-  rows[threadIdx.x] = row;
   uint32_t held[kOriginViews / 4];
 #pragma unroll
   for (int g = 0; g < kOriginViews / 4; ++g) {
     const int m4 = g_lo + 4 * g;
-    held[g] = (eligible && 4 * g < group_views && m4 < m_end) ? *reinterpret_cast<const uint32_t *>(classes + row + m4) : 0u;
-#pragma unroll
-    for (int q = 0; q < 4; ++q) tile[4 * g + q][threadIdx.x].origin = kNotWanted;
-  }
+    held[g] = (eligible && 4 * g < group_views && m4 < m_end) ? *reinterpret_cast<const uint32_t *>(marks + m4) : 0u;
+  }
+  if constexpr (RESIDUAL) {
+    uint32_t any = 0;
+#pragma unroll
+    for (int g = 0; g < kOriginViews / 4; ++g) any |= held[g] & (0x01010101u * COARSE_CHILDREN_WRITTEN);
+    if (__syncthreads_or(any != 0) == 0) return;
+  }
+  rows[threadIdx.x] = row;
+#pragma unroll
+  for (int q = 0; q < kOriginViews; ++q) tile[q][threadIdx.x].origin = kNotWanted;
+  double wxa, wya, wza;
+  brick_anchor(a, tk, bx, by, bz, wxa, wya, wza);
 #pragma unroll
   for (int g = 0; g < kOriginViews / 4; ++g) {
     const int m4 = g_lo + 4 * g;
@@ -626,55 +712,15 @@
     for (int q = 0; q < 4; ++q) {
       const int m = m4 + q;
       const uint8_t c = (uint8_t)(c4 >> (8 * q));
-      const bool want = eligible && m >= m_begin && m < m_end && (c & 0x1f) == (uint8_t)(BRICK_MIXED | (MIXED_FREE_OR_NODEPTH << 2));
+      const bool of_class = RESIDUAL ? (c & COARSE_CHILDREN_WRITTEN) != 0 : (c & 0x1f) == kWindowClass;
+      const bool want = eligible && m >= m_begin && m < m_end && of_class;
       if (__builtin_amdgcn_ballot_w64(want) == 0) continue;
-      WinPair wp;
-      wp.origin = kNotWanted;
-      wp.ax = wp.ay = wp.acz = 0.f;
-      if (cload(&a.win_recs[m].e_abs) < __builtin_inff()) {
-        const MapRec *src = maps + m;
-        const TileMapRec *tsrc = a.tile_maps + m;
-        const FootRec *fr = a.foot_recs + m;
-        const float(*scp)[4] = tk == 16 ? fr->s16 : fr->s8;
-        if (want) {
-          const double cza = ((cload(&src->rt[8]) * wxa + cload(&src->rt[9]) * wya) + cload(&src->rt[10]) * wza) + cload(&src->rt[11]);
-          const double hxa = __builtin_fma(cload(&tsrc->cpx), wxa, __builtin_fma(cload(&tsrc->cpy), wya, __builtin_fma(cload(&tsrc->cpz), wza, cload(&tsrc->cp0))));
-          const double hya = __builtin_fma(cload(&tsrc->cqx), wxa, __builtin_fma(cload(&tsrc->cqy), wya, __builtin_fma(cload(&tsrc->cqz), wza, cload(&tsrc->cq0))));
-          const float hx0 = (float)hxa, hy0 = (float)hya, z0 = (float)cza;
-          float umin = __builtin_inff(), umax = -__builtin_inff(), vmin = __builtin_inff(), vmax = -__builtin_inff();
-          float zmin = __builtin_inff(), zmax = -__builtin_inff();
-#pragma unroll
-          for (int cnr = 0; cnr < 8; ++cnr) {
-            const float z = z0 + cload(&scp[cnr][2]);
-            const float r = __builtin_amdgcn_rcpf(z);
-            const float u = (hx0 + cload(&scp[cnr][0])) * r, v = (hy0 + cload(&scp[cnr][1])) * r;
-            umin = __builtin_fminf(umin, u), umax = __builtin_fmaxf(umax, u);
-            vmin = __builtin_fminf(vmin, v), vmax = __builtin_fmaxf(vmax, v);
-            zmin = __builtin_fminf(zmin, z), zmax = __builtin_fmaxf(zmax, z);
-          }
-          const float umag = __builtin_fmaxf(__builtin_fmaxf(__builtin_fabsf(umin), __builtin_fabsf(umax)), __builtin_fmaxf(__builtin_fabsf(vmin), __builtin_fabsf(vmax)));
-          const float e = 2.0f * cload(&fr->ferr) * __builtin_amdgcn_rcpf(zmin) * (1.0f + 0x1p-20f) + (0x1p-19f * umag + 0x1p-12f);
-          const bool sane = zmin > 0.0f && zmax <= (float)(kWinCzRatio * (1.0 - 0x1p-20)) * zmin && umin > -65536.0f && umax < 65536.0f &&
-                            vmin > -65536.0f && vmax < 65536.0f && e < 0.25f;
-          if (sane) {
-            const int cxc = a.W / 2, cyc = a.H / 2;
-            const int x0 = (int)__builtin_ceilf(umin - 0.5f - e) + cxc, x1 = (int)__builtin_floorf(umax + 0.5f + e) + cxc;
-            const int y0 = (int)__builtin_ceilf(vmin - 0.5f - e) + cyc, y1 = (int)__builtin_floorf(vmax + 0.5f + e) + cyc;
-            if (x0 >= -kValidMargin && y0 >= -kValidMargin && x1 < a.W + kValidMargin && y1 < a.H + kValidMargin &&
-                x1 - x0 < kWindowCols && y1 - y0 < kWindowRows) {
-              wp.origin = (uint32_t)(x0 + kValidMargin) | ((uint32_t)(y0 + kValidMargin) << 16);
-              wp.ax = (float)(hxa - (double)(x0 - cxc) * cza);
-              wp.ay = (float)(hya - (double)(y0 - cyc) * cza);
-              wp.acz = z0;
-            }
-          }
-        }
-      }
       if (want) {
-        if (wp.origin != kNotWanted)
-          tile[4 * g + q][threadIdx.x] = wp;
+        WinPair wp;
+        if (pair_window<true>(a, maps, tk, m, wxa, wya, wza, wp))
+          tile[q + 4 * g][threadIdx.x] = wp;
         else
-          classes[row + m] = (uint8_t)(c | CLASS_NO_WINDOW);
+          classes[row + m] = RESIDUAL ? (uint8_t)(kWindowClass | CLASS_NO_WINDOW) : (uint8_t)(c | CLASS_NO_WINDOW);
       }
     }
   }
@@ -1012,8 +1058,8 @@
   return hipGetLastError();
 }
 
-hipError_t launch_window_origins(const TileArgs &a, const MapRec *maps_dev, int tk, uint8_t *classes, int general_k,
-                                 hipStream_t stream) {
+hipError_t launch_window_origins(const TileArgs &a, const MapRec *maps_dev, int tk, uint8_t *classes, const uint8_t *coarse,
+                                 int general_k, hipStream_t stream) {
   if (general_k || !a.win_origin || a.n_maps <= 0) return hipSuccess;
   const int bz_count = std::min(2 * a.super_z, a.bricks_z - 2 * a.sbz_first);
   const int64_t n_bricks = (int64_t)a.wbricks_x * a.wbricks_y * bz_count;
@@ -1023,10 +1069,18 @@
   int group_views = kOriginViews;
   while (group_views > 4 && brick_groups * ((span + group_views - 1) / group_views) < 2048) group_views >>= 1;
   const dim3 grid((unsigned)brick_groups, (unsigned)((span + group_views - 1) / group_views));
-  if (a.rotated)
-    hipLaunchKernelGGL((window_origin_kernel<true>), grid, dim3(256), 0, stream, a, maps_dev, tk, classes, a.win_origin, group_views);
+  const bool residual = !(a.flags & TILE_FLAG_ORIGINS_SEPARATE);
+#define DMI_LAUNCH_ORIGINS(R, S) \
+  hipLaunchKernelGGL((window_origin_kernel<R, S>), grid, dim3(256), 0, stream, a, maps_dev, tk, classes, coarse, a.win_origin, group_views)
+  if (a.rotated && residual)
+    DMI_LAUNCH_ORIGINS(true, true);
+  else if (a.rotated)
+    DMI_LAUNCH_ORIGINS(true, false);
+  else if (residual)
+    DMI_LAUNCH_ORIGINS(false, true);
   else
-    hipLaunchKernelGGL((window_origin_kernel<false>), grid, dim3(256), 0, stream, a, maps_dev, tk, classes, a.win_origin, group_views);
+    DMI_LAUNCH_ORIGINS(false, false);
+#undef DMI_LAUNCH_ORIGINS
   return hipGetLastError();
 }
 
@@ -1060,8 +1114,9 @@
   if (const char *env = getenv("DMI_QUERY_TILES")) q = atoi(env);
 #endif
   const bool wide = tk == 8;
+  WinPair *fine_origins = (general_k || (a.flags & TILE_FLAG_ORIGINS_SEPARATE)) ? nullptr : a.win_origin;
 #define DMI_LAUNCH_FINE_G(Q, C, R, G) \
-  hipLaunchKernelGGL((classify_kernel<Q, C, R, G>), fine_grid, dim3(256), 0, stream, a, maps_dev, P, tk, classes, coarse, group_views)
+  hipLaunchKernelGGL((classify_kernel<Q, C, R, G>), fine_grid, dim3(256), 0, stream, a, maps_dev, P, tk, classes, coarse, group_views, fine_origins)
 #define DMI_LAUNCH_FINE_R(Q, C, R)      \
   do {                                  \
     if (general_k)                      \
diff --git a/cudadepthmapintegration_amd/csrc/fusion_kernels.h b/cudadepthmapintegration_amd/csrc/fusion_kernels.h
--- a/cudadepthmapintegration_amd/csrc/fusion_kernels.h
+++ b/cudadepthmapintegration_amd/csrc/fusion_kernels.h
@@ -180,6 +180,7 @@
   TILE_FLAG_NO_INTERIOR = 1,
   TILE_FLAG_XCD_RUNS = 2,
   TILE_FLAG_COST_ORDER = 4,
+  TILE_FLAG_ORIGINS_SEPARATE = 8,
   TILE_FLAG_DBG_SKIP_WINDOW_PAIRS = 256,
   TILE_FLAG_DBG_ONLY_WINDOW_PAIRS = 512,
   TILE_FLAG_DBG_NO_WINDOW_LOADS = 1024
@@ -234,7 +235,8 @@
   VAR_NO_WINDOWS = 262144,
   VAR_WINDOWS_ALWAYS = 524288,
   VAR_COST_ORDER = 1048576,
-  VAR_NO_COST_ORDER = 2097152
+  VAR_NO_COST_ORDER = 2097152,
+  VAR_ORIGINS_SEPARATE = 4194304
 };
 
 constexpr int kMaxColumnHeight = 16;
@@ -259,8 +261,8 @@
                                int64_t n_maps, int W, int H, const PyramidDesc &desc, DepthTile *pyramids, uint8_t *valid, uint32_t *bits,
                                unsigned long long *counters, hipStream_t stream);
 hipError_t launch_build_pyramid_levels(int64_t n_maps, const PyramidDesc &desc, DepthTile *pyramids, hipStream_t stream);
-hipError_t launch_window_origins(const TileArgs &args, const MapRec *maps_dev, int tk, uint8_t *classes, int general_k,
-                                 hipStream_t stream);
+hipError_t launch_window_origins(const TileArgs &args, const MapRec *maps_dev, int tk, uint8_t *classes, const uint8_t *coarse,
+                                 int general_k, hipStream_t stream);
 hipError_t launch_classify_bricks(const TileArgs &args, const MapRec *maps_dev, const PyramidDesc &desc, int tk,
                                   uint8_t *classes, uint8_t *coarse, int general_k, hipStream_t stream);
 int64_t coarse_class_bytes(const TileArgs &args, int tk);
diff --git a/cudadepthmapintegration_amd/csrc/fusion_tile.hip b/cudadepthmapintegration_amd/csrc/fusion_tile.hip
--- a/cudadepthmapintegration_amd/csrc/fusion_tile.hip
+++ b/cudadepthmapintegration_amd/csrc/fusion_tile.hip
@@ -1320,7 +1320,7 @@
     const TileShape sh = tile_shape(cfg.variant, cfg.depth_is_f64 != 0, a.rotated != 0, cfg.general_k != 0);
     e = launch_classify_bricks(a, maps_dev, pyramid, sh.tk, const_cast<uint8_t *>(a.classes), coarse_classes, cfg.general_k, stream);
     if (e != hipSuccess) return e;
-    e = launch_window_origins(a, maps_dev, sh.tk, const_cast<uint8_t *>(a.classes), cfg.general_k, stream);
+    e = launch_window_origins(a, maps_dev, sh.tk, const_cast<uint8_t *>(a.classes), coarse_classes, cfg.general_k, stream);
     if (e != hipSuccess) return e;
 #ifdef DMI_TUNING
     if (const char *env = getenv("DMI_DEBUG_CLASS_REMAP")) {
diff --git a/include/dmi.h b/include/dmi.h
--- a/include/dmi.h
+++ b/include/dmi.h
@@ -141,6 +141,8 @@
 int dmi_get_mixed_reason_histogram(dmi_context *ctx, uint64_t out[8]);
 
 int dmi_get_window_pair_count(dmi_context *ctx, uint64_t *out);
+
+int dmi_get_pair_tables(dmi_context *ctx, uint8_t *classes, void *win_pairs, int64_t capacity_pairs, int64_t *bricks, int32_t *views);
 
 int dmi_get_view_paths(dmi_context *ctx, uint64_t out[6]);
 
```

Measured after the change: 2880. 0.99x the previous value.
